# kfjahnke/envutil

Hardware: AMD Instinct MI355X
Metric: Mpix/s reprojected (16K lat/lon->cubemap, b-spline-3) (higher is better)
Workload: dtype f32

## Files before the change

### envutil_amd/csrc/eu_render4.hip

```cpp
#include <cstdlib>
#include <cstdio>
#include <cstring>
#include <vector>
#include <algorithm>
#include "eu_packed_dev.h"

#define EU4_TW 16
#define EU4_TH 8
#define EU4_WAVES 4
#ifndef EU4_WAVES0
#define EU4_WAVES0 1
#define EU4_TEXELS 384
#define EU4_OCC0 4
#endif
#define EU4_SHARDS 1024
#define EU4_WL_SHARD(s) (16 * (s))
#define EU4_WL_DONE1 (16 * EU4_SHARDS)
#define EU4_WL_DYN(x) (16 * (EU4_SHARDS + 1 + (x)))
#define EU4_WL_ENTRIES (16 * (EU4_SHARDS + 16))
#define EU4_UNIT_ROWS 4
#define EU4_COL_FLOATS 8
#define EU4_MAX_PLANS 16

__device__ __forceinline__ void eu4_box_reduce(int &mn0, int &mn1, int &mx0, int &mx1)
{
#define EU4_RED(ctrl)                                        \
  "v_min_i32_dpp %0, %0, %0 " ctrl "\n\t"                    \
  "v_min_i32_dpp %1, %1, %1 " ctrl "\n\t"                    \
  "v_max_i32_dpp %2, %2, %2 " ctrl "\n\t"                    \
  "v_max_i32_dpp %3, %3, %3 " ctrl "\n\t"
  asm("s_nop 1\n\t"
      EU4_RED("row_shr:1 row_mask:0xf bank_mask:0xf")
      EU4_RED("row_shr:2 row_mask:0xf bank_mask:0xf")
      EU4_RED("row_shr:4 row_mask:0xf bank_mask:0xf")
      EU4_RED("row_shr:8 row_mask:0xf bank_mask:0xf")
      EU4_RED("row_bcast:15 row_mask:0xa bank_mask:0xf")
      EU4_RED("row_bcast:31 row_mask:0xc bank_mask:0xf")
      "s_nop 0"
      : "+v"(mn0), "+v"(mn1), "+v"(mx0), "+v"(mx1));
#undef EU4_RED
  mn0 = __builtin_amdgcn_readlane(mn0, 63); mn1 = __builtin_amdgcn_readlane(mn1, 63);
  mx0 = __builtin_amdgcn_readlane(mx0, 63); mx1 = __builtin_amdgcn_readlane(mx1, 63);
}

typedef __attribute__((address_space(3))) void *eu4_lds_void;
typedef const __attribute__((address_space(1))) void *eu4_gbl_void;

typedef float eu4_f4 __attribute__((ext_vector_type(4)));

__device__ __forceinline__ void eu4_dma_row(unsigned dst, unsigned voff, const char *sb)
{
  unsigned keep;
  asm volatile("s_mov_b32 %0, m0\n\t"
               "s_mov_b32 m0, %1\n\t"
               "s_nop 0\n\t"
               "global_load_lds_dwordx4 %2, %3\n\t"
               "s_mov_b32 m0, %0"
               : "=&s"(keep) : "s"(dst), "v"(voff), "s"(sb) : "memory");
}

struct eu4_plan {
  const float *atab_g;
  const int *tileplan;
  const float *coltab;
  int tiles16;
  const int *l2_rows;
  int l2_off[9];
  int l2_half;
  unsigned long long l2_magic;
  const int *l1_rows;
  int l1_off[9];
  unsigned long long l1_magic;
#ifdef EU5_STAMPS
  unsigned long long *stamps;
#endif
};

#ifdef EU5_STAMPS
#define EU5_STAMP(k) do { asm volatile("" ::: "memory"); st_[k] = __builtin_amdgcn_s_memtime(); asm volatile("" ::: "memory"); } while (0)
#else
#define EU5_STAMP(k) do { } while (0)
#endif

template <int NCH, int DEG, int PRJ>
__device__ __forceinline__ void eu4_tile(const eu_render_params &p, const eu4_plan &w, const float *atab,
                                         float *wtile, int tile_y, int x0, int lane)
{
  constexpr int TEX = 4;
  constexpr int order = DEG + 1;
  const eu_src_dev &s = p.src;
  const int lx = lane & 7, ly = lane >> 3;
  const int y = p.row_begin + tile_y * EU4_TH + ly;
  const bool yin = y < p.row_end;
  const int yc = yin ? y : p.row_end - 1;
  const float *rt = p.row + (long long)eu_frame_row(yc, p.band_shift, p.band_count, p.band_index) * EU_ROW_FLOATS;
  const int xa = x0 + 2 * lx, xb = xa + 1;
  const bool va = yin && xa < p.width, vb = yin && xb < p.width;
  const int xac = xa < p.width ? xa : p.width - 1, xbc = xb < p.width ? xb : p.width - 1;

  eu_f2 tx, ty, gy;
  eu_i2 hit, ok = { -1, -1 };
  int ixa, ixb;
  float wxa[order], wxb[order];
  eu_ray2 r;
  {
    const float A0 = rt[0], A1 = rt[1], A2 = rt[2], B0 = rt[3], B1 = rt[4], B2 = rt[5];
    const eu_f2 c0 = { p.col[xac], p.col[xbc] };
    if (p.form == EU_FORM_BCA) {
      const float C0 = rt[6], C1 = rt[7], C2 = rt[8];
      const float *colB = p.col + p.width;
      const eu_f2 c1 = { colB[xac], colB[xbc] };
      r.x = B0 * c0 + C0 * c1 + A0;
      r.y = B1 * c0 + C1 * c1 + A1;
      r.z = B2 * c0 + C2 * c1 + A2;
    } else {
      r.x = B0 * c0 + A0;
      r.y = B1 * c0 + A1;
      r.z = B2 * c0 + A2;
    }
    if (p.norm_mode == EU_NORM_DIV) {
      eu_f2 sqn = r.x * r.x; sqn = sqn + r.y * r.y; sqn = sqn + r.z * r.z;
      const eu_f2 n = { sqrtf(sqn.x), sqrtf(sqn.y) };
      r.x = r.x / n; r.y = r.y / n; r.z = r.z / n;
    }
  }
  asm volatile("s_waitcnt vmcnt(0)" ::: "memory");
  eu_f2 sx, sy;
  hit = eu_coord2_ok<PRJ>(s, r, sx, sy, atab, ok);
  const eu_f2 gx = eu_gate2_ok(sx, s.gate0, s.lower0, s.upper0, ok);
  gy = eu_gate2_ok(sy, s.gate1, s.lower1, s.upper1, ok);
  eu_f2 fx;
  if constexpr (DEG & 1) fx = (eu_f2){ floorf(gx.x), floorf(gx.y) };
  else fx = (eu_f2){ roundf(gx.x), roundf(gx.y) };
  tx = gx - fx;
  ixa = (int)fx.x; ixb = (int)fx.y;
  hit = hit & (eu_i2){ va ? -1 : 0, vb ? -1 : 0 };
  eu_f2 fy;
  if constexpr (DEG & 1) fy = (eu_f2){ floorf(gy.x), floorf(gy.y) };
  else fy = (eu_f2){ roundf(gy.x), roundf(gy.y) };
  ty = gy - fy;
  const int iya = (int)fy.x, iyb = (int)fy.y;

  int mnx = INT_MAX, mny = INT_MAX, mxx = INT_MIN, mxy = INT_MIN;
  if (hit.x) { mnx = ixa; mxx = ixa; mny = iya; mxy = iya; }
  if (hit.y) { mnx = min(mnx, ixb); mxx = max(mxx, ixb); mny = min(mny, iyb); mxy = max(mxy, iyb); }
  eu4_box_reduce(mnx, mny, mxx, mxy);
  const bool any = mnx != INT_MAX;
  const long long bw = (long long)mxx - mnx + order, bh = (long long)mxy - mny + order;
  const bool fits = bw <= 64 && bh <= EU4_TEXELS && bw * bh <= EU4_TEXELS;
  const bool clean = __ballot((hit.x && !ok.x) || (hit.y && !ok.y)) == 0ull;
  float *const orow = p.out + (long long)(yc - p.row_begin) * p.out_stride;
  if (any && !(fits && clean)) {
    if (lane == 0) {
      const int id = tile_y * w.tiles16 + x0 / EU4_TW;
      const int sh = (int)(((unsigned)id * 0x9E3779B1u) >> 22) & (EU4_SHARDS - 1);
      const int slot = atomicAdd(p.wl + EU4_WL_SHARD(sh), 1);
      p.wl[EU4_WL_ENTRIES + (size_t)slot * EU4_SHARDS + sh] = id;
    }
    return;
  }
  float qa[NCH], qb[NCH];
  if (any) {
    const int ibw = (int)bw, ibh = (int)bh;
    const unsigned lds_tile = (unsigned)(unsigned long long)(eu4_lds_void)wtile;
    if (lane < ibw) {
      const int bx0 = mnx - DEG / 2, by0 = mny - DEG / 2;
      const unsigned voff = (unsigned)(lane * NCH) * 4u;
      const char *sb = (const char *)(s.base + ((long long)by0 * s.es1 + (long long)bx0 * NCH));
      const long long step = s.es1 * 4;
      unsigned dst = lds_tile;
      const unsigned dstep = (unsigned)ibw * (TEX * 4u);
#pragma unroll 1
      for (int it = 0; it < ibh; it++) { eu4_dma_row(dst, voff, sb); sb += step; dst += dstep; }
    }
    eu_f2 wx[order], wy[order];
    float wya[order], wyb[order];
    if constexpr (DEG >= 2) {
      eu_weights2<DEG>(s.wm, ty, wy);
      eu_weights2<DEG>(s.wm, tx, wx);
    }
#pragma unroll
    for (int i = 0; i < order; i++) {
      if constexpr (DEG >= 2) {
        wya[i] = wy[i].x; wyb[i] = wy[i].y;
        wxa[i] = wx[i].x; wxb[i] = wx[i].y;
      } else {
        wya[i] = wyb[i] = 0.0f;
        wxa[i] = wxb[i] = 0.0f;
      }
    }
    const int oa = hit.x ? ((iya - mny) * ibw + (ixa - mnx)) * TEX : 0;
    const int ob = hit.y ? ((iyb - mny) * ibw + (ixb - mnx)) * TEX : 0;
    asm volatile("s_waitcnt vmcnt(0)" ::: "memory");
    eu_lptr lt = (eu_lptr)wtile;
    eu_accumulate1<NCH, DEG, TEX, int, eu_lptr>(lt + oa, ibw * TEX, wxa, wya, tx.x, ty.x, qa);
    eu_accumulate1<NCH, DEG, TEX, int, eu_lptr>(lt + ob, ibw * TEX, wxb, wyb, tx.y, ty.y, qb);
  } else {
#pragma unroll
    for (int c = 0; c < NCH; c++) { qa[c] = 0.0f; qb[c] = 0.0f; }
  }
  constexpr int ncol = (NCH == 2 || NCH == 4) ? NCH - 1 : NCH;
  const bool bright = s.brighten != 1.0f;
#pragma unroll
  for (int c = 0; c < NCH; c++) {
    float a = qa[c], bb = qb[c];
    if (bright && c < ncol) { a = a * s.brighten; bb = bb * s.brighten; }
    qa[c] = hit.x ? a : 0.0f;
    qb[c] = hit.y ? bb : 0.0f;
  }
  if (va) eu_put<NCH>(orow, xa, qa);
  if (vb) eu_put<NCH>(orow, xb, qb);
}

template <int NCH, int DEG, int PRJ>
__global__ __launch_bounds__(64 * EU4_WAVES0, EU4_OCC0) void eu_render4s_kernel(const eu_render_params p, const eu4_plan w)
{
  __shared__ __attribute__((aligned(16))) float tile_all[EU4_WAVES0 * EU4_TEXELS * 4];
  __shared__ __attribute__((aligned(16))) float atab[768];
  const int lane = threadIdx.x & 63;
  const int wave = __builtin_amdgcn_readfirstlane(threadIdx.x >> 6);
  float *const tile = tile_all + wave * (EU4_TEXELS * 4);
  if (PRJ != EU_CUBEMAP && wave == 0) {
    static_assert(EU_ATAN_TAB_FLOATS * 4 <= 3 * 1024, "three pieces");
#pragma unroll
    for (int i = 0; i < 3; i++)
      __builtin_amdgcn_global_load_lds((eu4_gbl_void)(w.atab_g + i * 256 + lane * 4),
                                       (eu4_lds_void)(atab + i * 256), 16, 0, 0);
  }
  const int tile_x = (int)(blockIdx.x >> 3) * EU4_WAVES0 + wave;
  const int tile_y = ((int)blockIdx.z * 8 + (int)(blockIdx.x & 7)) * EU4_UNIT_ROWS + (int)blockIdx.y;
  if (tile_y >= p.tiles_y) return;
  if constexpr (EU4_WAVES0 > 1) {
    asm volatile("s_waitcnt vmcnt(0)" ::: "memory");
    __syncthreads();
  }
  if (tile_x >= w.tiles16) return;
  eu4_tile<NCH, DEG, PRJ>(p, w, atab, tile, tile_y, tile_x * EU4_TW, lane);
}

template <int NCH, int DEG, int PRJ>
__device__ __forceinline__ void eu4_direct_tile(const eu_render_params &p, const float *atab, int tile_y, int x0, int lane)
{
  const eu_src_dev &s = p.src;
  const int lx = lane & 7, ly = lane >> 3;
  const int y = p.row_begin + tile_y * EU4_TH + ly;
  const bool yin = y < p.row_end;
  const int yc = yin ? y : p.row_end - 1;
  const float *rt = p.row + (long long)eu_frame_row(yc, p.band_shift, p.band_count, p.band_index) * EU_ROW_FLOATS;
  const int xa = x0 + 2 * lx, xb = xa + 1;
  const bool va = yin && xa < p.width, vb = yin && xb < p.width;
  const int xac = xa < p.width ? xa : p.width - 1, xbc = xb < p.width ? xb : p.width - 1;
  eu_ray2 ry;
  {
    const float A0 = rt[0], A1 = rt[1], A2 = rt[2], B0 = rt[3], B1 = rt[4], B2 = rt[5];
    const eu_f2 c0 = { p.col[xac], p.col[xbc] };
    if (p.form == EU_FORM_BCA) {
      const float C0 = rt[6], C1 = rt[7], C2 = rt[8];
      const float *colB = p.col + p.width;
      const eu_f2 c1 = { colB[xac], colB[xbc] };
      ry.x = B0 * c0 + C0 * c1 + A0;
      ry.y = B1 * c0 + C1 * c1 + A1;
      ry.z = B2 * c0 + C2 * c1 + A2;
    } else {
      ry.x = B0 * c0 + A0;
      ry.y = B1 * c0 + A1;
      ry.z = B2 * c0 + A2;
    }
    if (p.norm_mode == EU_NORM_DIV) {
      eu_f2 sqn = ry.x * ry.x; sqn = sqn + ry.y * ry.y; sqn = sqn + ry.z * ry.z;
      const eu_f2 n = { sqrtf(sqn.x), sqrtf(sqn.y) };
      ry.x = ry.x / n; ry.y = ry.y / n; ry.z = ry.z / n;
    }
  }
  eu_f2 sx, sy;
  eu_i2 hit = eu_coord2<PRJ>(s, ry, sx, sy, atab);
  hit = hit & (eu_i2){ va ? -1 : 0, vb ? -1 : 0 };
  float pxa[NCH], pxb[NCH];
  eu_eval2<NCH, DEG>(s, sx, sy, hit, pxa, pxb);
  float *const orow = p.out + (long long)(yc - p.row_begin) * p.out_stride;
  if (va) eu_put<NCH>(orow, xa, pxa);
  if (vb) eu_put<NCH>(orow, xb, pxb);
}

#include "eu_render5.h"

template <int DEG>
__global__ __launch_bounds__(256) void eu_colplan_kernel(const eu_render_params p, float *ct,
                                                         float A0, float A2, float B0, float B2)
{
  __shared__ __attribute__((aligned(16))) float atab[EU_ATAN_TAB_FLOATS];
  if (threadIdx.x < EU_ATAN_TAB_ENTRIES) eu_atan_tab_entry(threadIdx.x, atab + 8 * threadIdx.x);
  __syncthreads();
  constexpr int order = DEG + 1;
  const eu_src_dev &s = p.src;
  const int xa = 2 * (blockIdx.x * 256 + threadIdx.x), xb = xa + 1;
  if (xa >= p.width) return;
  const int xbc = xb < p.width ? xb : p.width - 1;
  const eu_f2 c0 = { p.col[xa], p.col[xbc] };
  const eu_f2 rx = B0 * c0 + A0, rz = B2 * c0 + A2;
  eu_i2 ok = { -1, -1 };
  const eu_f2 q2 = rx * rx + rz * rz;
  const eu_f2 qs = eu_sqrt2_ok(q2, ok);
  const eu_f2 lon = eu_atan2f_2_tab_ok(rx, rz, atab, 0, ok);
  eu_f2 i0 = { (float)((double)lon.x - s.tex_x0), (float)((double)lon.y - s.tex_x0) };
  if (s.cdiv_ok) i0 = eu_div2_const(i0, s.ext_w, s.rcp_ext_w);
  else i0 = i0 / s.ext_w;
  i0 = i0 * s.total_w; i0 = i0 - .5f;
  const eu_f2 sx = i0 - s.win_x_off;
  const eu_f2 gx = eu_gate2_ok(sx, s.gate0, s.lower0, s.upper0, ok);
  eu_f2 fx;
  if constexpr (DEG & 1) fx = (eu_f2){ floorf(gx.x), floorf(gx.y) };
  else fx = (eu_f2){ roundf(gx.x), roundf(gx.y) };
  const eu_f2 tx = gx - fx;
  eu_f2 wx[4];
#pragma unroll
  for (int i = 0; i < 4; i++) wx[i] = (eu_f2){ 0.0f, 0.0f };
  if constexpr (DEG >= 2) eu_weights2<DEG>(s.wm, tx, wx);
  float e[2][EU4_COL_FLOATS];
  e[0][0] = __int_as_float(ok.x ? (int)fx.x : INT_MIN);
  e[1][0] = __int_as_float(ok.y ? (int)fx.y : INT_MIN);
  e[0][1] = tx.x; e[1][1] = tx.y;
#pragma unroll
  for (int i = 0; i < 4; i++) { e[0][2 + i] = i < order ? wx[i].x : 0.0f; e[1][2 + i] = i < order ? wx[i].y : 0.0f; }
  e[0][6] = qs.x; e[1][6] = qs.y;
  e[0][7] = lon.x; e[1][7] = lon.y;
  float *o = ct + (size_t)xa * EU4_COL_FLOATS;
#pragma unroll
  for (int i = 0; i < EU4_COL_FLOATS; i++) o[i] = e[0][i];
  if (xb < p.width) {
#pragma unroll
    for (int i = 0; i < EU4_COL_FLOATS; i++) o[EU4_COL_FLOATS + i] = e[1][i];
  }
}

template <int NCH, int DEG, int PRJ>
__global__ __launch_bounds__(256, 4) void eu_render4d_kernel(const eu_render_params p, const eu4_plan w)
{
  __shared__ __attribute__((aligned(16))) float atab[EU_ATAN_TAB_FLOATS];
  if constexpr (PRJ != EU_CUBEMAP) {
    if (threadIdx.x < EU_ATAN_TAB_ENTRIES) eu_atan_tab_entry(threadIdx.x, atab + 8 * threadIdx.x);
  }
  const int lane = threadIdx.x & 63;
  const int wave = __builtin_amdgcn_readfirstlane(threadIdx.x >> 6);
  const int gid = blockIdx.x * EU4_WAVES + wave;
  const int sh = gid & (EU4_SHARDS - 1);
  const int nwork = __builtin_amdgcn_readfirstlane(
    __hip_atomic_load(p.wl + EU4_WL_SHARD(sh), __ATOMIC_RELAXED, __HIP_MEMORY_SCOPE_AGENT));
  __syncthreads();
#pragma unroll 1
  for (int k = gid / EU4_SHARDS; k < nwork; k += (int)(gridDim.x * EU4_WAVES / EU4_SHARDS)) {
    const int id = __builtin_amdgcn_readfirstlane(p.wl[EU4_WL_ENTRIES + (size_t)k * EU4_SHARDS + sh]);
    const int tile_y = id / w.tiles16;
    const int x0 = (id - tile_y * w.tiles16) * EU4_TW;
    eu4_direct_tile<NCH, DEG, PRJ>(p, atab, tile_y, x0, lane);
  }
  __shared__ int last;
  __syncthreads();
  if (threadIdx.x == 0) last = atomicAdd(p.wl + EU4_WL_DONE1, 1) == (int)gridDim.x - 1;
  __syncthreads();
  if (last) {
    for (int i = threadIdx.x; i <= EU4_SHARDS + 8; i += 256)
      __hip_atomic_store(p.wl + 16 * i, 0, __ATOMIC_RELAXED, __HIP_MEMORY_SCOPE_AGENT);
  }
}

#ifndef EU4_DIRECT_WGS
#define EU4_DIRECT_WGS 2048
#endif

template <int NCH, int DEG, int PRJ>
static int launch4_ndp(const eu_render_params &p, const eu4_plan &w, hipStream_t st)
{
  if constexpr (PRJ == EU_SPHERICAL) {
    static const int cus = [] {
      int dev = 0, n = 0;
      if (hipGetDevice(&dev) != hipSuccess) return 0;
      if (hipDeviceGetAttribute(&n, hipDeviceAttributeMultiprocessorCount, dev) != hipSuccess) return 0;
      return n;
    }();
    auto mag_ok = [](double v) { const double a = v < 0 ? -v : v; return a == 0.0 || (a >= 0x1p-20 && a <= 0x1p20); };
    const bool fast = p.form == EU_FORM_BA && p.norm_mode == EU_NORM_NONE && p.band_count <= 1 && p.src.brighten == 1.0f &&
                      p.src.always_hit && mag_ok(p.src.tex_x0) && mag_ok(p.src.tex_y0) && p.src.ext_w >= 0x1p-20f &&
                      p.src.ext_w <= 0x1p20f && p.src.ext_h >= 0x1p-20f && p.src.ext_h <= 0x1p20f && p.tab_finite;
    int per_cu = 0;
    if (fast) {
      static const int occ = [] { int n = 0; return hipOccupancyMaxActiveBlocksPerMultiprocessor(&n, eu_render5_kernel<NCH, DEG, PRJ, true>, 64 * EU5_WAVES, 0) == hipSuccess ? n : 0; }();
      per_cu = occ;
    } else {
      static const int occ = [] { int n = 0; return hipOccupancyMaxActiveBlocksPerMultiprocessor(&n, eu_render5_kernel<NCH, DEG, PRJ, false>, 64 * EU5_WAVES, 0) == hipSuccess ? n : 0; }();
      per_cu = occ;
    }
    const int wgs = (cus / 8) * 8 * per_cu;
    if (wgs <= 0) return -1;
    if (fast) hipLaunchKernelGGL((eu_render5_kernel<NCH, DEG, PRJ, true>), dim3((unsigned)wgs), dim3(64 * EU5_WAVES), 0, st, p, w);
    else hipLaunchKernelGGL((eu_render5_kernel<NCH, DEG, PRJ, false>), dim3((unsigned)wgs), dim3(64 * EU5_WAVES), 0, st, p, w);
  } else {
    const int units = (p.tiles_y + EU4_UNIT_ROWS - 1) / EU4_UNIT_ROWS;
    dim3 grid((unsigned)(8 * ((w.tiles16 + EU4_WAVES0 - 1) / EU4_WAVES0)), (unsigned)EU4_UNIT_ROWS, (unsigned)((units + 7) / 8));
    hipLaunchKernelGGL((eu_render4s_kernel<NCH, DEG, PRJ>), grid, dim3(64 * EU4_WAVES0), 0, st, p, w);
  }
  if (hipGetLastError() != hipSuccess) return -1;
  hipLaunchKernelGGL((eu_render4d_kernel<NCH, DEG, PRJ>), dim3(EU4_DIRECT_WGS), dim3(256), 0, st, p, w);
  if (hipGetLastError() != hipSuccess) {
    (void)hipMemsetAsync(p.wl, 0, EU4_WL_ENTRIES * sizeof(int), st);
    return -1;
  }
  return 0;
}

template <int NCH, int DEG>
static int launch4_nd(const eu_render_params &p, const eu4_plan &w, hipStream_t st)
{
  switch (p.src.prj) {
    case EU_SPHERICAL: return launch4_ndp<NCH, DEG, EU_SPHERICAL>(p, w, st);
    case EU_CUBEMAP: return launch4_ndp<NCH, DEG, EU_CUBEMAP>(p, w, st);
    case EU_BIATAN6: return launch4_ndp<NCH, DEG, EU_BIATAN6>(p, w, st);
  }
  return 1;
}

template <int NCH>
static int launch4_n(const eu_render_params &p, const eu4_plan &w, hipStream_t st)
{
  switch (p.src.degree) {
    case 1: return launch4_nd<NCH, 1>(p, w, st);
    case 2: return launch4_nd<NCH, 2>(p, w, st);
    case 3: return launch4_nd<NCH, 3>(p, w, st);
  }
  return 1;
}

extern "C" size_t eu_render4_worklist_ints(size_t ntiles)
{
  return EU4_WL_ENTRIES + ((ntiles + EU4_SHARDS - 1) / EU4_SHARDS) * EU4_SHARDS;
}
extern "C" size_t eu_render4_worklist_header_ints(void) { return EU4_WL_ENTRIES; }

extern "C" int eu_current_slot(void);
namespace {
struct plan_cache {
  std::vector<unsigned char> key;
  int *tileplan = nullptr; size_t tileplan_cap = 0;
  float *coltab = nullptr; size_t coltab_cap = 0;
  float *atab = nullptr;
  int planned_rows = 0;
  int *l2_rows = nullptr; size_t l2_cap = 0;
  int l2_off[9] = {};
  int *l1_rows = nullptr; size_t l1_cap = 0;
  int l1_off[9] = {};
  hipStream_t last_stream = nullptr;
} g4s[EU_MAX_SLOTS];
#define g4 (g4s[eu_current_slot()])

bool ensure_atab()
{
  if (g4.atab) return true;
  std::vector<float> tab(768, 0.0f);
  for (int i = 0; i < EU_ATAN_TAB_ENTRIES; i++) eu_atan_tab_entry(i, tab.data() + 8 * i);
  if (hipMalloc((void **)&g4.atab, tab.size() * sizeof(float)) != hipSuccess) return false;
  return hipMemcpy(g4.atab, tab.data(), tab.size() * sizeof(float), hipMemcpyHostToDevice) == hipSuccess;
}

template <int DEG>
void launch_colplan(const eu_render_params &p, float *ct, const float *k, hipStream_t st)
{
  hipLaunchKernelGGL((eu_colplan_kernel<DEG>), dim3((unsigned)((p.width + 511) / 512)), dim3(256), 0, st, p, ct,
                     k[0], k[1], k[2], k[3]);
}
}

extern "C" int eu_launch_render4(const eu_render_params *pp, const float *h_row, size_t h_row_floats,
                                 unsigned long long plan_gen, int only_if_worth, void *stream)
{
  eu_render_params p = *pp;
  if (p.twine || p.stage != 0 || p.form >= EU_FORM_FISH || p.src.has_lcp || p.nch_out != p.nch) return 1;
  if (p.norm_mode != EU_NORM_NONE && p.norm_mode != EU_NORM_DIV) return 1;
  if (p.src.prj != EU_SPHERICAL && p.src.prj != EU_CUBEMAP && p.src.prj != EU_BIATAN6) return 1;
  if (p.src.degree < 1 || p.src.degree > 3 || p.src.es0 != p.nch) return 1;
  if (p.nch != 3 && p.nch != 4) return 1;
  if (!p.wl) return 1;
  if (p.src.es1 * 4 >= (1ll << 31)) return 1;
  p.tiles_y = (p.row_end - p.row_begin + EU4_TH - 1) / EU4_TH;
  eu4_plan w;
  w.tiles16 = (p.width + EU4_TW - 1) / EU4_TW;
  if (w.tiles16 <= 0 || p.tiles_y <= 0) return 0;
  if (p.tiles_y > 65535 * 8 * EU4_UNIT_ROWS) return 1;
  hipStream_t st = (hipStream_t)stream;
  if (!ensure_atab()) return -1;
  w.atab_g = g4.atab;

  std::vector<unsigned char> key(sizeof(unsigned long long) + sizeof(eu_src_dev) + 8 * sizeof(int));
  {
    unsigned char *q = key.data();
    memcpy(q, &plan_gen, sizeof plan_gen); q += sizeof plan_gen;
    eu_src_dev sd = p.src; sd.base = nullptr;
    memcpy(q, &sd, sizeof sd); q += sizeof sd;
    const int v[8] = { p.width, p.row_begin, p.row_end, p.band_shift, p.band_count, p.band_index, p.form, p.norm_mode };
    memcpy(q, v, sizeof v);
  }
  if (p.src.prj == EU_SPHERICAL && key != g4.key) {
    std::vector<int> tp((size_t)p.tiles_y, -1);
    std::vector<float> plans;
    const bool can = p.src.prj == EU_SPHERICAL && p.form == EU_FORM_BA && p.norm_mode == EU_NORM_NONE && h_row;
    static const bool off = [] { const char *e = getenv("EU_HIP_COLPLAN"); return e && e[0] == '0'; }();
    if (can && !off) {
      for (int ty = 0; ty < p.tiles_y; ty++) {
        float k[4] = { 0, 0, 0, 0 };
        bool same = true;
        for (int ly = 0; ly < EU4_TH && same; ly++) {
          const int y = std::min(p.row_begin + ty * EU4_TH + ly, p.row_end - 1);
          const size_t fr = (size_t)eu_frame_row(y, p.band_shift, p.band_count, p.band_index) * EU_ROW_FLOATS;
          if (fr + 6 > h_row_floats) { same = false; break; }
          const float c[4] = { h_row[fr + 0], h_row[fr + 2], h_row[fr + 3], h_row[fr + 5] };
          if (ly == 0) memcpy(k, c, sizeof k);
          else same = memcmp(k, c, sizeof k) == 0;
        }
        if (!same) continue;
        int id = -1;
        for (size_t j = 0; j < plans.size() / 4 && id < 0; j++)
          if (memcmp(&plans[4 * j], k, sizeof k) == 0) id = (int)j;
        if (id < 0 && plans.size() / 4 < EU4_MAX_PLANS) {
          id = (int)(plans.size() / 4);
          plans.insert(plans.end(), k, k + 4);
        }
        tp[(size_t)ty] = id;
      }
    }
    if (g4.tileplan_cap < tp.size()) {
      if (g4.tileplan) (void)hipFree(g4.tileplan);
      g4.tileplan = nullptr; g4.tileplan_cap = 0;
      if (hipMalloc((void **)&g4.tileplan, tp.size() * sizeof(int)) != hipSuccess) return -1;
      g4.tileplan_cap = tp.size();
    }
    const size_t need = std::max<size_t>(1, plans.size() / 4) * (size_t)p.width * EU4_COL_FLOATS;
    if (g4.coltab_cap < need) {
      if (g4.coltab) (void)hipFree(g4.coltab);
      g4.coltab = nullptr; g4.coltab_cap = 0;
      if (hipMalloc((void **)&g4.coltab, need * sizeof(float)) != hipSuccess) return -1;
      g4.coltab_cap = need;
    }
    if (hipStreamSynchronize(st) != hipSuccess) return -1;
    if (g4.last_stream && g4.last_stream != st && hipStreamSynchronize(g4.last_stream) != hipSuccess) return -1;
    if (hipMemcpy(g4.tileplan, tp.data(), tp.size() * sizeof(int), hipMemcpyHostToDevice) != hipSuccess) return -1;
    g4.planned_rows = 0;
    for (int v : tp) g4.planned_rows += v >= 0;
    {
      std::vector<int> rows[8];
      for (int r = 0; r < p.tiles_y; r++) {
        const int m = r >> 1;
        const bool paired = 2 * m + 1 < p.tiles_y && tp[(size_t)2 * m] >= 0 && tp[(size_t)2 * m] == tp[(size_t)2 * m + 1];
        if (!paired) rows[(r / EU5_UNIT_ROWS) & 7].push_back(r);
      }
      std::vector<int> all;
      for (int x = 0; x < 8; x++) { g4.l2_off[x] = (int)all.size(); all.insert(all.end(), rows[x].begin(), rows[x].end()); }
      g4.l2_off[8] = (int)all.size();
      if (g4.l2_cap < all.size() + 1) {
        if (g4.l2_rows) (void)hipFree(g4.l2_rows);
        g4.l2_rows = nullptr; g4.l2_cap = 0;
        if (hipMalloc((void **)&g4.l2_rows, (all.size() + 1) * sizeof(int)) != hipSuccess) return -1;
        g4.l2_cap = all.size() + 1;
      }
      if (!all.empty() && hipMemcpy(g4.l2_rows, all.data(), all.size() * sizeof(int), hipMemcpyHostToDevice) != hipSuccess) return -1;
      std::vector<int> prs[8];
      for (int m = 0; 2 * m + 1 < p.tiles_y; m++)
        if (tp[(size_t)2 * m] >= 0 && tp[(size_t)2 * m] == tp[(size_t)2 * m + 1]) {
          auto &v = prs[(m / (EU5_UNIT_ROWS / 2)) & 7];
          v.push_back(m); v.push_back(tp[(size_t)2 * m]);
        }
      std::vector<int> all1;
      for (int x = 0; x < 8; x++) { g4.l1_off[x] = (int)all1.size() / 2; all1.insert(all1.end(), prs[x].begin(), prs[x].end()); }
      g4.l1_off[8] = (int)all1.size() / 2;
      if (g4.l1_cap < all1.size() + 2) {
        if (g4.l1_rows) (void)hipFree(g4.l1_rows);
        g4.l1_rows = nullptr; g4.l1_cap = 0;
        if (hipMalloc((void **)&g4.l1_rows, (all1.size() + 2) * sizeof(int)) != hipSuccess) return -1;
        g4.l1_cap = all1.size() + 2;
      }
      if (!all1.empty() && hipMemcpy(g4.l1_rows, all1.data(), all1.size() * sizeof(int), hipMemcpyHostToDevice) != hipSuccess) return -1;
    }
    for (size_t j = 0; j < plans.size() / 4; j++) {
      float *ct = g4.coltab + j * (size_t)p.width * EU4_COL_FLOATS;
      switch (p.src.degree) {
        case 1: launch_colplan<1>(p, ct, &plans[4 * j], st); break;
        case 2: launch_colplan<2>(p, ct, &plans[4 * j], st); break;
        default: launch_colplan<3>(p, ct, &plans[4 * j], st); break;
      }
      if (hipGetLastError() != hipSuccess) return -1;
    }
    g4.key.swap(key);
  }
  if (only_if_worth && p.src.prj == EU_SPHERICAL) {
    if (p.src.degree < 2 || g4.planned_rows * 2 < p.tiles_y) return 1;
  }
  w.tileplan = g4.tileplan;
  w.coltab = g4.coltab;
  w.l2_rows = g4.l2_rows;
  for (int x = 0; x < 9; x++) w.l2_off[x] = g4.l2_off[x];
  w.l2_half = (w.tiles16 + 1) / 2;
  w.l2_magic = (1ull << 40) / (unsigned long long)w.l2_half + 1;
  w.l1_rows = g4.l1_rows;
  for (int x = 0; x < 9; x++) w.l1_off[x] = g4.l1_off[x];
  w.l1_magic = (1ull << 40) / (unsigned long long)w.tiles16 + 1;
  g4.last_stream = st;
#ifdef EU5_STAMPS
  static unsigned long long *d_st = nullptr; static size_t st_cap = 0; static int dumps = 0;
  const size_t ntile_st = (size_t)w.tiles16 * p.tiles_y * 8;
  const size_t nst = ntile_st + 8192 * 4;
  if (st_cap < nst) { if (d_st) (void)hipFree(d_st); if (hipMalloc((void **)&d_st, nst * 8) != hipSuccess) return -1; st_cap = nst; }
  (void)hipMemsetAsync(d_st, 0, nst * 8, st);
  w.stamps = d_st;
  int rc_ = p.nch == 3 ? launch4_n<3>(p, w, st) : p.nch == 4 ? launch4_n<4>(p, w, st) : 1;
  if (rc_ == 0 && dumps < 2 && nst >= 8 * 4096) {
    dumps++;
    std::vector<unsigned long long> h(nst);
    (void)hipStreamSynchronize(st);
    (void)hipMemcpy(h.data(), d_st, nst * 8, hipMemcpyDeviceToHost);
    double acc[32][8] = {}; size_t cnt[32] = {};
    for (size_t t = 0; t < ntile_st / 8; t++) {
      const unsigned long long *q = &h[t * 8];
      if (!q[0] || !q[7]) continue;
      const int cls = (int)(q[1] & 31);
      cnt[cls]++;
      acc[cls][0] += (double)(q[2] - q[0]); acc[cls][1] += (double)(q[3] - q[2]);
      if (q[4]) { acc[cls][2] += (double)(q[4] - q[3]); acc[cls][3] += (double)(q[5] - q[4]); acc[cls][4] += (double)(q[6] - q[5]); }
      acc[cls][5] += (double)(q[7] - q[6]); acc[cls][6] += (double)(q[7] - q[0]);
    }
    {
      double mn = 1e30, mx = 0, sum = 0, l1 = 0, first = 1e30, last = 0; size_t nw = 0;
      for (size_t k = 0; k < 8192; k++) {
        const unsigned long long *q = &h[ntile_st + k * 4];
        if (!q[3]) continue;
        const double d = (double)(q[2] - q[0]);
        mn = std::min(mn, d); mx = std::max(mx, d); sum += d; l1 += (double)(q[1] - q[0]); nw++;
        first = std::min(first, (double)q[0]); last = std::max(last, (double)q[2]);
      }
      if (nw) fprintf(stderr, "eu5 waves: %zu, cycles per wave min %.0f avg %.0f max %.0f, first loop avg %.0f, first start .. last end %.0f\n",
                      nw, mn, sum / nw, mx, l1 / nw, last - first);
    }
    for (int c = 0; c < 32; c++) if (cnt[c])
      fprintf(stderr, "eu5 stamps: hoist %d npass %2d tiles %8zu | coords %7.0f box %6.0f dma-issue+weights %6.0f dma-wait %6.0f taps(all passes) %6.0f store %5.0f | tile %7.0f (100 MHz ticks? s_memtime)\n",
              c >> 4, (c & 15) - 1, cnt[c], acc[c][0] / cnt[c], acc[c][1] / cnt[c], acc[c][2] / cnt[c], acc[c][3] / cnt[c], acc[c][4] / cnt[c], acc[c][5] / cnt[c], acc[c][6] / cnt[c]);
  }
  return rc_;
#else
  switch (p.nch) {
    case 3: return launch4_n<3>(p, w, st);
    case 4: return launch4_n<4>(p, w, st);
  }
  return 1;
#endif
}
```

### envutil_amd/csrc/eu_render5.h

```cpp
#define EU5_WAVES 4
#ifndef EU5_TEXELS
#define EU5_TEXELS 576
#endif
#ifndef EU5_OCC
#define EU5_OCC 4
#endif
#ifndef EU5_UNIT_ROWS
#define EU5_UNIT_ROWS 4
#endif

__device__ __forceinline__ int eu4_shard_of(int id)
{
  return (int)(((unsigned)id * 0x9E3779B1u) >> 22) & (EU4_SHARDS - 1);
}

typedef const __attribute__((address_space(3))) eu4_f4 *eu5_l4ptr;

template <int NCH, int DEG>
__device__ __forceinline__ void eu5_taps(eu_lptr lt, int a, int b, int pitch, const eu_f2 *wx, const eu_f2 *wy,
                                         eu_f2 tx, eu_f2 ty, eu_f2 &rga, eu_f2 &bxa, eu_f2 &rgb, eu_f2 &bxb)
{
  constexpr int order = DEG + 1;
  if constexpr (DEG == 1) {
    const eu_f2 wl0 = 1.0f - tx, wr0 = tx, wl1 = 1.0f - ty, wr1 = ty;
    const eu4_f4 a00 = *(eu5_l4ptr)(lt + a), a01 = *(eu5_l4ptr)(lt + a + 4);
    const eu4_f4 a10 = *(eu5_l4ptr)(lt + a + pitch), a11 = *(eu5_l4ptr)(lt + a + pitch + 4);
    const eu4_f4 b00 = *(eu5_l4ptr)(lt + b), b01 = *(eu5_l4ptr)(lt + b + 4);
    const eu4_f4 b10 = *(eu5_l4ptr)(lt + b + pitch), b11 = *(eu5_l4ptr)(lt + b + pitch + 4);
    {
      const eu_f2 l0 = { wl0.x, wl0.x }, r0 = { wr0.x, wr0.x }, l1 = { wl1.x, wl1.x }, r1 = { wr1.x, wr1.x };
      eu_f2 s = a00.xy * l0; s = s + a01.xy * r0; s = s * l1;
      eu_f2 u = a10.xy * l0; u = u + a11.xy * r0; rga = s + u * r1;
      s = a00.zw * l0; s = s + a01.zw * r0; s = s * l1;
      u = a10.zw * l0; u = u + a11.zw * r0; bxa = s + u * r1;
    }
    {
      const eu_f2 l0 = { wl0.y, wl0.y }, r0 = { wr0.y, wr0.y }, l1 = { wl1.y, wl1.y }, r1 = { wr1.y, wr1.y };
      eu_f2 s = b00.xy * l0; s = s + b01.xy * r0; s = s * l1;
      eu_f2 u = b10.xy * l0; u = u + b11.xy * r0; rgb = s + u * r1;
      s = b00.zw * l0; s = s + b01.zw * r0; s = s * l1;
      u = b10.zw * l0; u = u + b11.zw * r0; bxb = s + u * r1;
    }
  } else {
#pragma unroll
    for (int j = 0; j < order; j++) {
      eu4_f4 ta[order], tb[order];
#pragma unroll
      for (int i = 0; i < order; i++) {
        ta[i] = *(eu5_l4ptr)(lt + a + j * pitch + 4 * i);
        tb[i] = *(eu5_l4ptr)(lt + b + j * pitch + 4 * i);
      }
      const eu_f2 w0a = { wx[0].x, wx[0].x }, w0b = { wx[0].y, wx[0].y };
      eu_f2 ra = ta[0].xy * w0a, qa = ta[0].zw * w0a, rb = tb[0].xy * w0b, qb = tb[0].zw * w0b;
#pragma unroll
      for (int i = 1; i < order; i++) {
        const eu_f2 wa = { wx[i].x, wx[i].x }, wb = { wx[i].y, wx[i].y };
        ra = EU_MAD2(wa, ta[i].xy, ra); qa = EU_MAD2(wa, ta[i].zw, qa);
        rb = EU_MAD2(wb, tb[i].xy, rb); qb = EU_MAD2(wb, tb[i].zw, qb);
      }
      const eu_f2 ya = { wy[j].x, wy[j].x }, yb = { wy[j].y, wy[j].y };
      if (j == 0) { rga = ra * ya; bxa = qa * ya; rgb = rb * yb; bxb = qb * yb; }
      else { rga = EU_MAD2(ra, ya, rga); bxa = EU_MAD2(qa, ya, bxa); rgb = EU_MAD2(rb, yb, rgb); bxb = EU_MAD2(qb, yb, bxb); }
    }
  }
}

__device__ __forceinline__ void eu5_box_reduce(int &q0, int &q1, int &q2, int &q3, int &h0, int &h1, int &h2, int &h3)
{
#define EU5_RED(ctrl)                                        \
  "v_min_i32_dpp %0, %0, %0 " ctrl "\n\t"                    \
  "v_min_i32_dpp %1, %1, %1 " ctrl "\n\t"                    \
  "v_max_i32_dpp %2, %2, %2 " ctrl "\n\t"                    \
  "v_max_i32_dpp %3, %3, %3 " ctrl "\n\t"
  asm("s_nop 1\n\t"
      EU5_RED("row_shr:1 row_mask:0xf bank_mask:0xf")
      EU5_RED("row_shr:2 row_mask:0xf bank_mask:0xf")
      EU5_RED("row_shr:4 row_mask:0xf bank_mask:0xf")
      EU5_RED("row_shr:8 row_mask:0xf bank_mask:0xf")
      "v_mov_b32 %4, %0\n\tv_mov_b32 %5, %1\n\tv_mov_b32 %6, %2\n\tv_mov_b32 %7, %3\n\t"
      "v_min_i32_dpp %4, %0, %4 row_bcast:15 row_mask:0xa bank_mask:0xf\n\t"
      "v_min_i32_dpp %5, %1, %5 row_bcast:15 row_mask:0xa bank_mask:0xf\n\t"
      "v_max_i32_dpp %6, %2, %6 row_bcast:15 row_mask:0xa bank_mask:0xf\n\t"
      "v_max_i32_dpp %7, %3, %7 row_bcast:15 row_mask:0xa bank_mask:0xf\n\t"
      "s_nop 0"
      : "+v"(q0), "+v"(q1), "+v"(q2), "+v"(q3), "=&v"(h0), "=&v"(h1), "=&v"(h2), "=&v"(h3));
#undef EU5_RED
}

struct eu5_box { int mnx, mny, mxx, mxy; };

struct eu5_divtab_t { unsigned v[65]; };
static constexpr eu5_divtab_t eu5_make_divtab()
{
  eu5_divtab_t t = {};
  t.v[0] = 0;
  for (unsigned w = 1; w <= 64; w++) t.v[w] = ((65536u + w - 1) / w) | ((64u / w) << 24);
  return t;
}
__constant__ const eu5_divtab_t eu5_divtab = eu5_make_divtab();

__device__ __forceinline__ eu5_box eu5_box_at(int a, int b, int c, int d, int lane)
{
  eu5_box r;
  r.mnx = __builtin_amdgcn_readlane(a, lane); r.mny = __builtin_amdgcn_readlane(b, lane);
  r.mxx = __builtin_amdgcn_readlane(c, lane); r.mxy = __builtin_amdgcn_readlane(d, lane);
  return r;
}
__device__ __forceinline__ eu5_box eu5_box_join(const eu5_box &a, const eu5_box &b)
{
  eu5_box r = { min(a.mnx, b.mnx), min(a.mny, b.mny), max(a.mxx, b.mxx), max(a.mxy, b.mxy) };
  return r;
}
template <int ORDER>
__device__ __forceinline__ int eu5_box_fits(const eu5_box &b)
{
  if (b.mnx == INT_MAX) return -1;
  const unsigned bw = (unsigned)b.mxx - (unsigned)b.mnx + ORDER, bh = (unsigned)b.mxy - (unsigned)b.mny + ORDER;
  return bw <= 64u && bh <= (unsigned)EU5_TEXELS && bw * bh <= (unsigned)EU5_TEXELS;
}

__device__ __forceinline__ eu_f2 eu5_gate2(eu_f2 c, int kind, float lower, float upper)
{
  if (kind == 0) {
    eu_f2 r = c;
    r = eu_sel2(c < lower, (eu_f2){ lower, lower }, r);
    r = eu_sel2(c > upper, (eu_f2){ upper, upper }, r);
    return r;
  }
  eu_f2 cc = c - lower;
  if (kind == 1) cc = eu_abs2(cc);
  return cc + lower;
}

__device__ __forceinline__ int eu5_out_of_range3(float a, float b, float c)
{
  const float hi = __builtin_fmaxf(__builtin_fmaxf(__builtin_fabsf(a), __builtin_fabsf(b)), __builtin_fabsf(c));
  const float lo = __builtin_fminf(__builtin_fminf(__builtin_fabsf(a), __builtin_fabsf(b)), __builtin_fabsf(c));
  return (hi <= 0x1p40f && lo >= 0x1p-40f) ? 0 : -1;
}

struct eu5_tab8 { eu_f2 c0; float A0, A1, A2, B0, B1, B2; };

template <bool FAST>
__device__ __forceinline__ void eu5_load8(const eu_render_params &p, int tile_y, int x0, int lane, eu5_tab8 &T)
{
  const int pr = lane & 3, rw = (lane >> 2) & 7, hf = lane >> 5;
  const int y = p.row_begin + tile_y * EU4_TH + rw;
  const int yc = y < p.row_end ? y : p.row_end - 1;
  const float *rt = p.row + (long long)(FAST ? yc : eu_frame_row(yc, p.band_shift, p.band_count, p.band_index)) * EU_ROW_FLOATS;
  const int xa = x0 + 8 * hf + 2 * pr, xb = xa + 1;
  const int xac = xa < p.width ? xa : p.width - 1, xbc = xb < p.width ? xb : p.width - 1;
  T.A0 = rt[0]; T.A1 = rt[1]; T.A2 = rt[2]; T.B0 = rt[3]; T.B1 = rt[4]; T.B2 = rt[5];
  T.c0 = (eu_f2){ p.col[xac], p.col[xbc] };
}

template <int NCH, int DEG, int PRJ, bool HOIST, bool FAST, bool PRE = false>
__device__ __forceinline__ void eu5_tile(const eu_render_params &p, const eu4_plan &w, const float *atab,
                                         float *wtile, const float *ct, int tile_y, int x0, int lane,
                                         const eu5_tab8 *T = nullptr, bool have_n = false, int ty_n = 0, int x0_n = 0,
                                         eu5_tab8 *Tn = nullptr)
{
  static_assert(!PRE || (!HOIST && FAST), "the prefetching form exists for plain FAST tiles");
  constexpr int TEX = 4;
  constexpr int order = DEG + 1;
  const eu_src_dev &s = p.src;
#ifdef EU5_STAMPS
  unsigned long long st_[8] = { 0, 0, 0, 0, 0, 0, 0, 0 };
#endif
  EU5_STAMP(0);
  const int pr = lane & 3, rw = (lane >> 2) & 7, hf = lane >> 5;
  const int y = p.row_begin + tile_y * EU4_TH + rw;
  const bool yin = y < p.row_end;
  const int yc = yin ? y : p.row_end - 1;
  const float *rt = p.row + (long long)(FAST ? yc : eu_frame_row(yc, p.band_shift, p.band_count, p.band_index)) * EU_ROW_FLOATS;
  const int xa = x0 + 8 * hf + 2 * pr, xb = xa + 1;
  const bool va = yin && xa < p.width, vb = yin && xb < p.width;
  const int xac = xa < p.width ? xa : p.width - 1, xbc = xb < p.width ? xb : p.width - 1;

  eu_f2 tx, ty, gy;
  eu_i2 hit, ok = { -1, -1 };
  int ixa, ixb;
  eu_f2 wx[order], wy[order];
  constexpr bool LEAN = FAST && PRJ == EU_SPHERICAL;
  if constexpr (LEAN) {
    hit = (eu_i2){ -1, -1 };
    eu_i2 big0 = { 0, 0 }, big1 = { 0, 0 };
    eu_f2 lat;
    if constexpr (HOIST) {
      const float4 *ea = (const float4 *)(ct + (size_t)xac * EU4_COL_FLOATS);
      const float4 *eb = (const float4 *)(ct + (size_t)xbc * EU4_COL_FLOATS);
      const float4 a0 = ea[0], a1 = ea[1], b0 = eb[0], b1 = eb[1];
      const float A1 = rt[1], B1 = rt[4];
      const eu_f2 c0 = { p.col[xac], p.col[xbc] };
      const eu_f2 ryy = B1 * c0 + A1;
      ixa = __float_as_int(a0.x); ixb = __float_as_int(b0.x);
      tx = (eu_f2){ a0.y, b0.y };
      if constexpr (DEG >= 2) {
        wx[0] = (eu_f2){ a0.z, b0.z }; wx[1] = (eu_f2){ a0.w, b0.w }; wx[2] = (eu_f2){ a1.x, b1.x };
        if constexpr (DEG == 3) wx[3] = (eu_f2){ a1.y, b1.y };
      }
      const eu_f2 qs = { a1.z, b1.z };
      ok = (eu_i2){ (ixa != INT_MIN ? -1 : 0) & ~eu5_out_of_range3(ryy.x, qs.x, qs.x),
                    (ixb != INT_MIN ? -1 : 0) & ~eu5_out_of_range3(ryy.y, qs.y, qs.y) };
      lat = eu_atan2f_2_lean(ryy, qs, atab, 1, big0);
    } else {
      float A0, A1, A2, B0, B1, B2;
      eu_f2 c0;
      if constexpr (PRE) { A0 = T->A0; A1 = T->A1; A2 = T->A2; B0 = T->B0; B1 = T->B1; B2 = T->B2; c0 = T->c0; }
      else {
        A0 = rt[0]; A1 = rt[1]; A2 = rt[2]; B0 = rt[3]; B1 = rt[4]; B2 = rt[5];
        c0 = (eu_f2){ p.col[xac], p.col[xbc] };
      }
      const eu_f2 rx = B0 * c0 + A0, ry = B1 * c0 + A1, rz = B2 * c0 + A2;
      ok = (eu_i2){ ~eu5_out_of_range3(rx.x, ry.x, rz.x), ~eu5_out_of_range3(rx.y, ry.y, rz.y) };
      const eu_f2 q2 = rx * rx + rz * rz;
      const eu_f2 qs = eu_sqrt2_safe(q2);
      lat = eu_atan2f_2_lean(ry, qs, atab, 1, big0);
      const eu_f2 lon = eu_atan2f_2_lean(rx, rz, atab, 0, big1);
      eu_f2 i0 = { (float)((double)lon.x - s.tex_x0), (float)((double)lon.y - s.tex_x0) };
      if (s.cdiv_ok) i0 = eu_div2_const(i0, s.ext_w, s.rcp_ext_w);
      else i0 = eu_div2_rr(i0, s.ext_w, eu_rcp_refined(s.ext_w));
      i0 = i0 * s.total_w; i0 = i0 - .5f;
      const eu_f2 sx = i0 - s.win_x_off;
      const eu_f2 gx = eu5_gate2(sx, s.gate0, s.lower0, s.upper0);
      eu_f2 fx;
      if constexpr (DEG & 1) fx = (eu_f2){ floorf(gx.x), floorf(gx.y) };
      else fx = (eu_f2){ roundf(gx.x), roundf(gx.y) };
      tx = gx - fx;
      ixa = (int)fx.x; ixb = (int)fx.y;
    }
    ok = ok & ~(big0 | big1);
    eu_f2 i1 = { (float)((double)lat.x - s.tex_y0), (float)((double)lat.y - s.tex_y0) };
    if (s.cdiv_ok) i1 = eu_div2_const(i1, s.ext_h, s.rcp_ext_h);
    else i1 = eu_div2_rr(i1, s.ext_h, eu_rcp_refined(s.ext_h));
    i1 = i1 * s.total_h; i1 = i1 - .5f;
    const eu_f2 sy = i1 - s.win_y_off;
    gy = eu5_gate2(sy, s.gate1, s.lower1, s.upper1);
  } else if constexpr (HOIST) {
    const float4 *ea = (const float4 *)(ct + (size_t)xac * EU4_COL_FLOATS);
    const float4 *eb = (const float4 *)(ct + (size_t)xbc * EU4_COL_FLOATS);
    const float4 a0 = ea[0], a1 = ea[1], b0 = eb[0], b1 = eb[1];
    const float A1 = rt[1], B1 = rt[4];
    const eu_f2 c0 = { p.col[xac], p.col[xbc] };
    const eu_f2 ryy = B1 * c0 + A1;
    ixa = __float_as_int(a0.x); ixb = __float_as_int(b0.x);
    ok = ok & (eu_i2){ ixa != INT_MIN ? -1 : 0, ixb != INT_MIN ? -1 : 0 };
    tx = (eu_f2){ a0.y, b0.y };
    if constexpr (DEG >= 2) {
      wx[0] = (eu_f2){ a0.z, b0.z }; wx[1] = (eu_f2){ a0.w, b0.w }; wx[2] = (eu_f2){ a1.x, b1.x };
      if constexpr (DEG == 3) wx[3] = (eu_f2){ a1.y, b1.y };
    }
    const eu_f2 qs = { a1.z, b1.z };
    const eu_f2 lat = eu_atan2f_2_tab_ok(ryy, qs, atab, 1, ok);
    hit = (eu_i2){ -1, -1 };
    if (!FAST && !s.always_hit) {
      const eu_f2 lon = { a1.w, b1.w };
      hit = (lon >= s.wex0) & (lon <= s.wex1) & (lat >= s.wex2) & (lat <= s.wex3);
    }
    eu_f2 i1 = { (float)((double)lat.x - s.tex_y0), (float)((double)lat.y - s.tex_y0) };
    if (FAST || s.cdiv_ok) i1 = eu_div2_const(i1, s.ext_h, s.rcp_ext_h);
    else i1 = i1 / s.ext_h;
    i1 = i1 * s.total_h; i1 = i1 - .5f;
    const eu_f2 sy = i1 - s.win_y_off;
    gy = eu_gate2_ok(sy, s.gate1, s.lower1, s.upper1, ok);
  } else {
    eu_ray2 r;
    {
      float A0, A1, A2, B0, B1, B2;
      eu_f2 c0;
      if constexpr (PRE) { A0 = T->A0; A1 = T->A1; A2 = T->A2; B0 = T->B0; B1 = T->B1; B2 = T->B2; c0 = T->c0; }
      else {
        A0 = rt[0]; A1 = rt[1]; A2 = rt[2]; B0 = rt[3]; B1 = rt[4]; B2 = rt[5];
        c0 = (eu_f2){ p.col[xac], p.col[xbc] };
      }
      if (!FAST && p.form == EU_FORM_BCA) {
        const float C0 = rt[6], C1 = rt[7], C2 = rt[8];
        const float *colB = p.col + p.width;
        const eu_f2 c1 = { colB[xac], colB[xbc] };
        r.x = B0 * c0 + C0 * c1 + A0;
        r.y = B1 * c0 + C1 * c1 + A1;
        r.z = B2 * c0 + C2 * c1 + A2;
      } else {
        r.x = B0 * c0 + A0;
        r.y = B1 * c0 + A1;
        r.z = B2 * c0 + A2;
      }
      if (!FAST && p.norm_mode == EU_NORM_DIV) {
        eu_f2 sqn = r.x * r.x; sqn = sqn + r.y * r.y; sqn = sqn + r.z * r.z;
        const eu_f2 n = { sqrtf(sqn.x), sqrtf(sqn.y) };
        r.x = r.x / n; r.y = r.y / n; r.z = r.z / n;
      }
    }
    eu_f2 sx, sy;
    hit = eu_coord2_ok<PRJ, FAST>(s, r, sx, sy, atab, ok);
    const eu_f2 gx = eu_gate2_ok(sx, s.gate0, s.lower0, s.upper0, ok);
    gy = eu_gate2_ok(sy, s.gate1, s.lower1, s.upper1, ok);
    eu_f2 fx;
    if constexpr (DEG & 1) fx = (eu_f2){ floorf(gx.x), floorf(gx.y) };
    else fx = (eu_f2){ roundf(gx.x), roundf(gx.y) };
    tx = gx - fx;
    ixa = (int)fx.x; ixb = (int)fx.y;
  }
  hit = hit & (eu_i2){ va ? -1 : 0, vb ? -1 : 0 };
  eu_f2 fy;
  if constexpr (DEG & 1) fy = (eu_f2){ floorf(gy.x), floorf(gy.y) };
  else fy = (eu_f2){ roundf(gy.x), roundf(gy.y) };
  ty = gy - fy;
  const int iya = (int)fy.x, iyb = (int)fy.y;
#ifdef EU5_STAMPS
  asm volatile("" : : "v"(iya), "v"(iyb), "v"(ixa), "v"(ixb));
#endif
  EU5_STAMP(2);

  int q0 = INT_MAX, q1 = INT_MAX, q2 = INT_MIN, q3 = INT_MIN, h0, h1, h2, h3;
  if (hit.x) { q0 = ixa; q2 = ixa; q1 = iya; q3 = iya; }
  if (hit.y) { q0 = min(q0, ixb); q2 = max(q2, ixb); q1 = min(q1, iyb); q3 = max(q3, iyb); }
  eu5_box_reduce(q0, q1, q2, q3, h0, h1, h2, h3);
  const eu5_box full = eu5_box_join(eu5_box_at(h0, h1, h2, h3, 31), eu5_box_at(h0, h1, h2, h3, 63));
  bool clean = __ballot((hit.x && !ok.x) || (hit.y && !ok.y)) == 0ull;
  if constexpr (LEAN) {
    const int cw = (int)(s.upper0 + 0.5f), ch = (int)(s.upper1 + 0.5f);
    if (full.mnx != INT_MAX) {
      if (s.gate0 == 2 && full.mnx < 0) clean = false;
      if (s.gate0 != 0 && full.mxx >= cw - 1) clean = false;
      if (s.gate1 == 2 && full.mny < 0) clean = false;
      if (s.gate1 != 0 && full.mxy >= ch - 1) clean = false;
    }
  }
  int npass = 1;
  const int f = eu5_box_fits<order>(full);
  if (f < 0) npass = 0;
  else if (f == 0) {
    npass = 2;
    if (eu5_box_fits<order>(eu5_box_at(h0, h1, h2, h3, 31)) == 0 || eu5_box_fits<order>(eu5_box_at(h0, h1, h2, h3, 63)) == 0) {
      npass = 4;
      if (eu5_box_fits<order>(eu5_box_at(q0, q1, q2, q3, 15)) == 0 || eu5_box_fits<order>(eu5_box_at(q0, q1, q2, q3, 31)) == 0 ||
          eu5_box_fits<order>(eu5_box_at(q0, q1, q2, q3, 47)) == 0 || eu5_box_fits<order>(eu5_box_at(q0, q1, q2, q3, 63)) == 0)
        npass = -1;
    }
  }
  EU5_STAMP(3);
  float *const orow = p.out + (long long)(yc - p.row_begin) * p.out_stride;
  if (npass < 0 || (npass > 0 && !clean)) {
    if (lane == 0) {
      const int id = tile_y * w.tiles16 + x0 / EU4_TW;
      const int sh = eu4_shard_of(id);
      const int slot = atomicAdd(p.wl + EU4_WL_SHARD(sh), 1);
      p.wl[EU4_WL_ENTRIES + (size_t)slot * EU4_SHARDS + sh] = id;
    }
    if constexpr (PRE) { if (have_n) eu5_load8<FAST>(p, ty_n, x0_n, lane, *Tn); }
    return;
  }
  eu_f2 rga = { 0.0f, 0.0f }, bxa = { 0.0f, 0.0f }, rgb = { 0.0f, 0.0f }, bxb = { 0.0f, 0.0f };
  if (npass > 0) {
    const unsigned lds_tile = (unsigned)(unsigned long long)(eu4_lds_void)wtile;
    const int grp = npass == 1 ? 0 : npass == 2 ? hf : (lane >> 4);
#pragma unroll 1
    for (int pi = 0; pi < npass; pi++) {
      eu5_box bx = full;
      if (npass > 1) {
        const int ln = npass == 2 ? 31 + 32 * pi : 15 + 16 * pi;
        const eu5_box bh = eu5_box_at(h0, h1, h2, h3, ln), bq = eu5_box_at(q0, q1, q2, q3, ln);
        bx = npass == 2 ? bh : bq;
      }
      if (bx.mnx == INT_MAX) continue;
      const int ibw = bx.mxx - bx.mnx + order, ibh = bx.mxy - bx.mny + order;
      {
        const unsigned tv = eu5_divtab.v[ibw];
        const int k = (int)(tv >> 24);
        const unsigned r = ((unsigned)lane * (tv & 0x1ffffu)) >> 16, c = (unsigned)lane - r * (unsigned)ibw;
        const int bx0 = bx.mnx - DEG / 2, by0 = bx.mny - DEG / 2;
        const unsigned pitchb = (unsigned)(s.es1 * 4);
        const unsigned voff = r * pitchb + c * (NCH * 4u);
        const char *sb = (const char *)(s.base + ((long long)by0 * s.es1 + (long long)bx0 * NCH));
        const unsigned long long step = (unsigned long long)k * pitchb;
        unsigned dst = lds_tile;
        const unsigned dstep = (unsigned)(k * ibw) * (TEX * 4u);
        int left = ibh;
        if ((int)r < k) {
#pragma unroll 1
          for (; left >= k; left -= k) { eu4_dma_row(dst, voff, sb); sb += step; dst += dstep; }
        }
        left = ibh % k;
        if ((int)r < left) {
          const int full = ibh / k;
          eu4_dma_row(lds_tile + (unsigned)full * dstep, voff,
                      (const char *)(s.base + ((long long)by0 * s.es1 + (long long)bx0 * NCH)) + (unsigned long long)full * step);
        }
      }
      if (pi == 0) {
        if constexpr (DEG >= 2) {
          eu_weights2<DEG>(s.wm, ty, wy);
          if constexpr (!HOIST) eu_weights2<DEG>(s.wm, tx, wx);
        }
      }
      const bool mine = grp == pi;
      const int oa = (mine && hit.x) ? ((iya - bx.mny) * ibw + (ixa - bx.mnx)) * TEX : 0;
      const int ob = (mine && hit.y) ? ((iyb - bx.mny) * ibw + (ixb - bx.mnx)) * TEX : 0;
      if (pi == 0) EU5_STAMP(4);
      asm volatile("s_waitcnt vmcnt(0)" ::: "memory");
      if (pi == 0) EU5_STAMP(5);
      if (mine) eu5_taps<NCH, DEG>((eu_lptr)wtile, oa, ob, ibw * TEX, wx, wy, tx, ty, rga, bxa, rgb, bxb);
    }
  }
#ifdef EU5_STAMPS
  asm volatile("" : : "v"(rga), "v"(bxa), "v"(rgb), "v"(bxb));
#endif
  EU5_STAMP(6);
  float qa[4] = { rga.x, rga.y, bxa.x, bxa.y }, qb[4] = { rgb.x, rgb.y, bxb.x, bxb.y };
  constexpr int ncol = (NCH == 2 || NCH == 4) ? NCH - 1 : NCH;
  const bool bright = !FAST && s.brighten != 1.0f;
#pragma unroll
  for (int c = 0; c < NCH; c++) {
    float a = qa[c], bb = qb[c];
    if (bright && c < ncol) { a = a * s.brighten; bb = bb * s.brighten; }
    qa[c] = hit.x ? a : 0.0f;
    qb[c] = hit.y ? bb : 0.0f;
  }
  if constexpr (PRE) {
    if (have_n) eu5_load8<FAST>(p, ty_n, x0_n, lane, *Tn);
    __builtin_amdgcn_sched_barrier(0);
  }
  if (va) eu_put<NCH>(orow, xa, qa);
  if (vb) eu_put<NCH>(orow, xb, qb);
  EU5_STAMP(7);
#ifdef EU5_STAMPS
  if (lane == 0 && w.stamps) {
    unsigned long long *o = w.stamps + ((size_t)tile_y * w.tiles16 + x0 / EU4_TW) * 8;
    st_[1] = (unsigned long long)(npass + 1) | (HOIST ? 16ull : 0ull);
#pragma unroll
    for (int k = 0; k < 8; k++) o[k] = st_[k];
  }
#endif
}



template <int NCH, int DEG>
__device__ __forceinline__ void eu5_stage(const eu_src_dev &s, const eu5_box &bx, unsigned lds_tile, int lane)
{
  constexpr int order = DEG + 1;
  const int ibw = bx.mxx - bx.mnx + order, ibh = bx.mxy - bx.mny + order;
  const unsigned tv = eu5_divtab.v[ibw];
  const int k = (int)(tv >> 24);
  const unsigned r = ((unsigned)lane * (tv & 0x1ffffu)) >> 16, c = (unsigned)lane - r * (unsigned)ibw;
  const int bx0 = bx.mnx - DEG / 2, by0 = bx.mny - DEG / 2;
  const unsigned pitchb = (unsigned)(s.es1 * 4);
  const unsigned voff = r * pitchb + c * (NCH * 4u);
  const char *const sb0 = (const char *)(s.base + ((long long)by0 * s.es1 + (long long)bx0 * NCH));
  const unsigned long long step = (unsigned long long)k * pitchb;
  const unsigned dstep = (unsigned)(k * ibw) * 16u;
  if ((int)r < k) {
    const char *sb = sb0;
    unsigned dst = lds_tile;
#pragma unroll 1
    for (int left = ibh; left >= k; left -= k) { eu4_dma_row(dst, voff, sb); sb += step; dst += dstep; }
  }
  if ((int)r < ibh % k) {
    const int full = ibh / k;
    eu4_dma_row(lds_tile + (unsigned)full * dstep, voff, sb0 + (unsigned long long)full * step);
  }
}

struct eu5_tab16 {
  eu4_f4 a0, a1, b0, b1;
  eu_f2 c0;
  float A1A, B1A, A1B, B1B;
};

__device__ __forceinline__ void eu5_load16(const eu_render_params &p, const float *ct, int tile_y, int x0, int lane, eu5_tab16 &T)
{
  const int pr = lane & 3, rw = (lane >> 2) & 7, hf = lane >> 5;
  const int yA = p.row_begin + tile_y * EU4_TH + rw, yB = yA + EU4_TH;
  const int ycA = yA < p.row_end ? yA : p.row_end - 1, ycB = yB < p.row_end ? yB : p.row_end - 1;
  const float *rtA = p.row + (long long)ycA * EU_ROW_FLOATS, *rtB = p.row + (long long)ycB * EU_ROW_FLOATS;
  const int xa = x0 + 8 * hf + 2 * pr, xb = xa + 1;
  const int xac = xa < p.width ? xa : p.width - 1, xbc = xb < p.width ? xb : p.width - 1;
  const eu4_f4 *ea = (const eu4_f4 *)(ct + (size_t)xac * EU4_COL_FLOATS);
  const eu4_f4 *eb = (const eu4_f4 *)(ct + (size_t)xbc * EU4_COL_FLOATS);
  T.a0 = ea[0]; T.a1 = ea[1]; T.b0 = eb[0]; T.b1 = eb[1];
  T.A1A = rtA[1]; T.B1A = rtA[4]; T.A1B = rtB[1]; T.B1B = rtB[4];
  T.c0 = (eu_f2){ p.col[xac], p.col[xbc] };
}

template <int NCH, int DEG>
__device__ __forceinline__ bool eu5_tile16h(const eu_render_params &p, const eu4_plan &w, const float *atab,
                                            float *wtile, const eu5_tab16 &T, int tile_y, int x0, int lane,
                                            bool have_n, const float *ct_n, int ty_n, int x0_n, eu5_tab16 &Tn)
{
  constexpr int order = DEG + 1;
  const eu_src_dev &s = p.src;
#ifdef EU5_STAMPS
  unsigned long long st_[8] = { 0, 0, 0, 0, 0, 0, 0, 0 };
#endif
  EU5_STAMP(0);
  const int pr = lane & 3, rw = (lane >> 2) & 7, hf = lane >> 5;
  const int yA = p.row_begin + tile_y * EU4_TH + rw, yB = yA + EU4_TH;
  const bool yinA = yA < p.row_end, yinB = yB < p.row_end;
  const int ycA = yinA ? yA : p.row_end - 1, ycB = yinB ? yB : p.row_end - 1;
  const int xa = x0 + 8 * hf + 2 * pr, xb = xa + 1;
  const bool vxa = xa < p.width, vxb = xb < p.width;
  const eu4_f4 a0 = T.a0, a1 = T.a1, b0 = T.b0, b1 = T.b1;
  const eu_f2 c0 = T.c0;
  const eu_f2 ryA = T.B1A * c0 + T.A1A, ryB = T.B1B * c0 + T.A1B;
  const int ixa = __float_as_int(a0.x), ixb = __float_as_int(b0.x);
  eu_f2 wx[order];
  const eu_f2 tx = { a0.y, b0.y };
  if constexpr (DEG >= 2) {
    wx[0] = (eu_f2){ a0.z, b0.z }; wx[1] = (eu_f2){ a0.w, b0.w }; wx[2] = (eu_f2){ a1.x, b1.x };
    if constexpr (DEG == 3) wx[3] = (eu_f2){ a1.y, b1.y };
  }
  const eu_f2 qs = { a1.z, b1.z };
  eu_i2 bigA = { 0, 0 }, bigB = { 0, 0 };
  int bad = ((ixa != INT_MIN && ixb != INT_MIN) ? 0 : -1) |
            eu5_out_of_range3(ryA.x, qs.x, ryB.x) | eu5_out_of_range3(ryA.y, qs.y, ryB.y);
  const eu_f2 latA = eu_atan2f_2_lean(ryA, qs, atab, 1, bigA);
  const eu_f2 latB = eu_atan2f_2_lean(ryB, qs, atab, 1, bigB);
  bad |= bigA.x | bigA.y | bigB.x | bigB.y;
  const float rr = s.cdiv_ok ? 0.0f : eu_rcp_refined(s.ext_h);
  eu_f2 iA = { (float)((double)latA.x - s.tex_y0), (float)((double)latA.y - s.tex_y0) };
  eu_f2 iB = { (float)((double)latB.x - s.tex_y0), (float)((double)latB.y - s.tex_y0) };
  if (s.cdiv_ok) { iA = eu_div2_const(iA, s.ext_h, s.rcp_ext_h); iB = eu_div2_const(iB, s.ext_h, s.rcp_ext_h); }
  else { iA = eu_div2_rr(iA, s.ext_h, rr); iB = eu_div2_rr(iB, s.ext_h, rr); }
  iA = iA * s.total_h; iA = iA - .5f; iB = iB * s.total_h; iB = iB - .5f;
  const eu_f2 gyA = eu5_gate2(iA - s.win_y_off, s.gate1, s.lower1, s.upper1);
  const eu_f2 gyB = eu5_gate2(iB - s.win_y_off, s.gate1, s.lower1, s.upper1);
  eu_f2 fyA, fyB;
  if constexpr (DEG & 1) { fyA = (eu_f2){ floorf(gyA.x), floorf(gyA.y) }; fyB = (eu_f2){ floorf(gyB.x), floorf(gyB.y) }; }
  else { fyA = (eu_f2){ roundf(gyA.x), roundf(gyA.y) }; fyB = (eu_f2){ roundf(gyB.x), roundf(gyB.y) }; }
  const eu_f2 tyA = gyA - fyA, tyB = gyB - fyB;
  const int iyAa = (int)fyA.x, iyAb = (int)fyA.y, iyBa = (int)fyB.x, iyBb = (int)fyB.y;
  const bool hAa = yinA && vxa, hAb = yinA && vxb, hBa = yinB && vxa, hBb = yinB && vxb;

#ifdef EU5_STAMPS
  asm volatile("" : : "v"(iyAa), "v"(iyAb), "v"(iyBa), "v"(iyBb));
#endif
  EU5_STAMP(2);
  int q0 = INT_MAX, q1 = INT_MAX, q2 = INT_MIN, q3 = INT_MIN, h0, h1, h2, h3;
  if (hAa) { q0 = ixa; q2 = ixa; q1 = iyAa; q3 = iyAa; }
  if (hAb) { q0 = min(q0, ixb); q2 = max(q2, ixb); q1 = min(q1, iyAb); q3 = max(q3, iyAb); }
  if (hBa) { q0 = min(q0, ixa); q2 = max(q2, ixa); q1 = min(q1, iyBa); q3 = max(q3, iyBa); }
  if (hBb) { q0 = min(q0, ixb); q2 = max(q2, ixb); q1 = min(q1, iyBb); q3 = max(q3, iyBb); }
  eu5_box_reduce(q0, q1, q2, q3, h0, h1, h2, h3);
  eu5_box bx = eu5_box_join(eu5_box_at(h0, h1, h2, h3, 31), eu5_box_at(h0, h1, h2, h3, 63));
  bool fast = __ballot(bad != 0 && (hAa || hAb || hBa || hBb)) == 0ull;
  if (bx.mnx != INT_MAX) {
    const int cw = (int)(s.upper0 + 0.5f), ch = (int)(s.upper1 + 0.5f);
    if (s.gate0 == 2 && bx.mnx < 0) fast = false;
    if (s.gate0 != 0 && bx.mxx >= cw - 1) fast = false;
    if (s.gate1 == 2 && bx.mny < 0) fast = false;
    if (s.gate1 != 0 && bx.mxy >= ch - 1) fast = false;
    if (eu5_box_fits<order>(bx) != 1) fast = false;
  }
  if (bx.mnx == INT_MAX || !fast) {
    if (have_n) eu5_load16(p, ct_n, ty_n, x0_n, lane, Tn);
    return bx.mnx == INT_MAX;
  }
  bx.mnx = __builtin_amdgcn_readfirstlane(bx.mnx); bx.mny = __builtin_amdgcn_readfirstlane(bx.mny);
  bx.mxx = __builtin_amdgcn_readfirstlane(bx.mxx); bx.mxy = __builtin_amdgcn_readfirstlane(bx.mxy);
  const unsigned lds_tile = (unsigned)(unsigned long long)(eu4_lds_void)wtile;
  EU5_STAMP(3);
  eu5_stage<NCH, DEG>(s, bx, lds_tile, lane);
  eu_f2 wyA[order], wyB[order];
  if constexpr (DEG >= 2) { eu_weights2<DEG>(s.wm, tyA, wyA); eu_weights2<DEG>(s.wm, tyB, wyB); }
  const int ibw = bx.mxx - bx.mnx + order;
  const int oAa = hAa ? ((iyAa - bx.mny) * ibw + (ixa - bx.mnx)) * 4 : 0, oAb = hAb ? ((iyAb - bx.mny) * ibw + (ixb - bx.mnx)) * 4 : 0;
  const int oBa = hBa ? ((iyBa - bx.mny) * ibw + (ixa - bx.mnx)) * 4 : 0, oBb = hBb ? ((iyBb - bx.mny) * ibw + (ixb - bx.mnx)) * 4 : 0;
  EU5_STAMP(4);
  asm volatile("s_waitcnt vmcnt(0)" ::: "memory");
  EU5_STAMP(5);
  __builtin_amdgcn_sched_barrier(0);
  eu_f2 rga, bxa, rgb, bxb;
  eu5_taps<NCH, DEG>((eu_lptr)wtile, oAa, oAb, ibw * 4, wx, wyA, tx, tyA, rga, bxa, rgb, bxb);
  asm volatile("" : "+v"(rga), "+v"(bxa), "+v"(rgb), "+v"(bxb));
  {
    float qa[4] = { rga.x, rga.y, bxa.x, bxa.y }, qb[4] = { rgb.x, rgb.y, bxb.x, bxb.y };
    float *const orow = p.out + (long long)(ycA - p.row_begin) * p.out_stride;
    if (hAa) eu_put<NCH>(orow, xa, qa);
    if (hAb) eu_put<NCH>(orow, xb, qb);
  }
  EU5_STAMP(6);
  __builtin_amdgcn_sched_barrier(0);
  eu5_taps<NCH, DEG>((eu_lptr)wtile, oBa, oBb, ibw * 4, wx, wyB, tx, tyB, rga, bxa, rgb, bxb);
  asm volatile("" : "+v"(rga), "+v"(bxa), "+v"(rgb), "+v"(bxb));
  if (have_n) eu5_load16(p, ct_n, ty_n, x0_n, lane, Tn);
  __builtin_amdgcn_sched_barrier(0);
  {
    float qa[4] = { rga.x, rga.y, bxa.x, bxa.y }, qb[4] = { rgb.x, rgb.y, bxb.x, bxb.y };
    float *const orow = p.out + (long long)(ycB - p.row_begin) * p.out_stride;
    if (hBa) eu_put<NCH>(orow, xa, qa);
    if (hBb) eu_put<NCH>(orow, xb, qb);
  }
  EU5_STAMP(7);
#ifdef EU5_STAMPS
  if (lane == 0 && w.stamps) {
    unsigned long long *o = w.stamps + ((size_t)tile_y * w.tiles16 + x0 / EU4_TW) * 8;
    st_[1] = 6ull | 16ull;
#pragma unroll
    for (int k = 0; k < 8; k++) o[k] = st_[k];
  }
#endif
  return true;
}

template <int UNIT>
struct eu5_iter {
  int ul, ry, rx;
  int du, dy, dx;
  int xcd, units, tiles16;
  __device__ __forceinline__ void start(int t0, int K)
  {
    const int per_unit = UNIT * tiles16;
    ul = t0 / per_unit;
    ry = (t0 - ul * per_unit) / tiles16;
    rx = t0 - ul * per_unit - ry * tiles16;
    du = K / per_unit; dy = (K - du * per_unit) / tiles16; dx = K - du * per_unit - dy * tiles16;
  }
  __device__ __forceinline__ void step()
  {
    rx += dx; ry += dy; ul += du;
    if (rx >= tiles16) { rx -= tiles16; ry++; }
    if (ry >= UNIT) { ry -= UNIT; ul++; }
  }
  __device__ __forceinline__ bool done() const { return ul * 8 + xcd >= units; }
  __device__ __forceinline__ int row() const { return (ul * 8 + xcd) * UNIT + ry; }
  __device__ __forceinline__ int col() const
  {
    const unsigned h = ((unsigned)row() * 0x9E3779B1u) >> 16;
    int c = rx + (int)((h * (unsigned)tiles16) >> 16);
    if (c >= tiles16) c -= tiles16;
    return c;
  }
};

typedef const __attribute__((address_space(4))) int *eu5_cint;
__device__ __forceinline__ int eu5_pair_plan(const int *tileplan, int tiles_y, int m)
{
  if (2 * m + 1 >= tiles_y) return -1;
  const eu5_cint tp = (eu5_cint)tileplan;
  const int a = tp[2 * m], b = tp[2 * m + 1];
  return a == b ? a : -1;
}

template <int NCH, int DEG, int PRJ, bool FAST>
__global__ __launch_bounds__(64 * EU5_WAVES, EU5_OCC) void eu_render5_kernel(const eu_render_params p, const eu4_plan w)
{
  __shared__ __attribute__((aligned(16))) float tile_all[EU5_WAVES * EU5_TEXELS * 4];
  __shared__ __attribute__((aligned(16))) float atab[768];
  const int lane0 = threadIdx.x & 63;
  const int wave = __builtin_amdgcn_readfirstlane(threadIdx.x >> 6);
  float *const tile = tile_all + wave * (EU5_TEXELS * 4);
  if (PRJ != EU_CUBEMAP && wave == 0) {
#pragma unroll
    for (int i = 0; i < 3; i++)
      __builtin_amdgcn_global_load_lds((eu4_gbl_void)(w.atab_g + i * 256 + lane0 * 4),
                                       (eu4_lds_void)(atab + i * 256), 16, 0, 0);
    asm volatile("s_waitcnt vmcnt(0)" ::: "memory");
  }
  __syncthreads();
#ifdef EU5_STAMPS
  const unsigned long long ws0 = __builtin_amdgcn_s_memtime();
  unsigned long long ws1 = ws0;
#endif
  const int xcd = (int)(blockIdx.x & 7);
  const int K = (int)(gridDim.x >> 3) * EU5_WAVES;
  const int t0 = (int)(blockIdx.x >> 3) * EU5_WAVES + wave;
  constexpr bool PAIRS = FAST && PRJ == EU_SPHERICAL;
  if constexpr (PAIRS) {
    const int n1 = (w.l1_off[xcd + 1] - w.l1_off[xcd]) * w.tiles16;
    const eu5_cint rows1 = (eu5_cint)w.l1_rows + 2 * w.l1_off[xcd];
    int pos1 = t0;
    auto seek = [&](int &m, int &tcol, int &plan) -> bool {
      if (pos1 >= n1) return false;
      const int r = (int)(((unsigned long long)(unsigned)pos1 * w.l1_magic) >> 40);
      m = rows1[2 * r]; plan = rows1[2 * r + 1];
      const unsigned h = ((unsigned)m * 0x9E3779B1u) >> 16;
      int c = pos1 - r * w.tiles16 + (int)((h * (unsigned)w.tiles16) >> 16);
      if (c >= w.tiles16) c -= w.tiles16;
      tcol = c;
      pos1 += K;
      return true;
    };
    int m_a = 0, col_a = 0, plan_a = -1, m_b = 0, col_b = 0, plan_b = -1;
    bool have_a = seek(m_a, col_a, plan_a), have_b = false;
    eu5_tab16 Ta, Tb;
    if (have_a) eu5_load16(p, w.coltab + (size_t)plan_a * p.width * EU4_COL_FLOATS, 2 * m_a, col_a * EU4_TW, lane0, Ta);
    auto fallback = [&](int m, int tcol, int lane) {
      if (lane < 2) {
        const int id = (2 * m + lane) * w.tiles16 + tcol;
        const int sh = eu4_shard_of(id);
        const int slot = atomicAdd(p.wl + EU4_WL_SHARD(sh), 1);
        p.wl[EU4_WL_ENTRIES + (size_t)slot * EU4_SHARDS + sh] = id;
      }
    };
#pragma unroll 1
    while (have_a) {
      {
        have_b = seek(m_b, col_b, plan_b);
        int lane = lane0;
        asm volatile("" : "+v"(lane));
        const float *ct_n = w.coltab + (size_t)(have_b ? plan_b : 0) * p.width * EU4_COL_FLOATS;
        if (!eu5_tile16h<NCH, DEG>(p, w, atab, tile, Ta, 2 * m_a, col_a * EU4_TW, lane, have_b, ct_n, 2 * m_b, col_b * EU4_TW, Tb))
          fallback(m_a, col_a, lane);
      }
      if (!have_b) break;
      {
        have_a = seek(m_a, col_a, plan_a);
        int lane = lane0;
        asm volatile("" : "+v"(lane));
        const float *ct_n = w.coltab + (size_t)(have_a ? plan_a : 0) * p.width * EU4_COL_FLOATS;
        if (!eu5_tile16h<NCH, DEG>(p, w, atab, tile, Tb, 2 * m_b, col_b * EU4_TW, lane, have_a, ct_n, 2 * m_a, col_a * EU4_TW, Ta))
          fallback(m_b, col_b, lane);
      }
    }
  }
#ifdef EU5_STAMPS
  ws1 = __builtin_amdgcn_s_memtime();
#endif
  eu5_iter<EU5_UNIT_ROWS> it;
  it.xcd = xcd; it.tiles16 = w.tiles16;
  it.units = (p.tiles_y + EU5_UNIT_ROWS - 1) / EU5_UNIT_ROWS;
  it.start(t0, K);
  if constexpr (PAIRS) {
    int *const queue = p.wl + EU4_WL_DYN(xcd);
    const int nbatch = (w.l2_off[xcd + 1] - w.l2_off[xcd]) * w.l2_half;
    const eu5_cint rows2 = (eu5_cint)w.l2_rows + w.l2_off[xcd];
    auto take = [&]() -> int {
      int v = 0;
      if (lane0 == 0) v = atomicAdd(queue, 1);
      return v;
    };
    auto decode = [&](int j, int &ty, int &tcol) -> bool {
      if (j >= nbatch) return false;
      const int r = (int)(((unsigned long long)(unsigned)j * w.l2_magic) >> 40);
      ty = rows2[r]; tcol = 2 * (j - r * w.l2_half);
      return true;
    };
    int ty_a = 0, col_a = 0, ty_n = 0, col_n = 0;
    bool have = decode(__builtin_amdgcn_readfirstlane(take()), ty_a, col_a);
    eu5_tab8 Ta, Tb;
    if (have) eu5_load8<FAST>(p, ty_a, col_a * EU4_TW, lane0, Ta);
#pragma unroll 1
    while (have) {
      const int jn_lane = take();
      const bool second = col_a + 1 < w.tiles16;
      {
        int lane = lane0;
        asm volatile("" : "+v"(lane));
        eu5_tile<NCH, DEG, PRJ, false, FAST, true>(p, w, atab, tile, nullptr, ty_a, col_a * EU4_TW, lane, &Ta, second, ty_a,
                                                   (col_a + 1) * EU4_TW, &Tb);
      }
      const bool have_n = decode(__builtin_amdgcn_readfirstlane(jn_lane), ty_n, col_n);
      if (second) {
        int lane = lane0;
        asm volatile("" : "+v"(lane));
        eu5_tile<NCH, DEG, PRJ, false, FAST, true>(p, w, atab, tile, nullptr, ty_a, (col_a + 1) * EU4_TW, lane, &Tb, have_n, ty_n,
                                                   col_n * EU4_TW, &Ta);
      } else if (have_n) eu5_load8<FAST>(p, ty_n, col_n * EU4_TW, lane0, Ta);
      ty_a = ty_n; col_a = col_n; have = have_n;
    }
  } else {
    int plan_n = (it.done() || it.row() >= p.tiles_y) ? -2 : (PRJ == EU_SPHERICAL ? ((eu5_cint)w.tileplan)[it.row()] : -1);
#pragma unroll 1
    while (!it.done()) {
      const int tile_y = it.row(), tcol = it.col(), plan = plan_n;
      it.step();
      plan_n = (it.done() || it.row() >= p.tiles_y) ? -2 : (PRJ == EU_SPHERICAL ? ((eu5_cint)w.tileplan)[it.row()] : -1);
      if (plan == -2) continue;
      int lane = lane0;
      asm volatile("" : "+v"(lane));
      if (plan >= 0)
        eu5_tile<NCH, DEG, PRJ, PRJ == EU_SPHERICAL, FAST>(p, w, atab, tile, w.coltab + (size_t)plan * p.width * EU4_COL_FLOATS,
                                                            tile_y, tcol * EU4_TW, lane);
      else
        eu5_tile<NCH, DEG, PRJ, false, FAST>(p, w, atab, tile, nullptr, tile_y, tcol * EU4_TW, lane);
    }
  }
#ifdef EU5_STAMPS
  if (lane0 == 0 && w.stamps) {
    unsigned long long *o = w.stamps + (size_t)w.tiles16 * p.tiles_y * 8 + ((size_t)blockIdx.x * EU5_WAVES + wave) * 4;
    o[0] = ws0; o[1] = ws1; o[2] = __builtin_amdgcn_s_memtime(); o[3] = 1;
  }
#endif
}
```

### include/eu_hip.h

```cpp
#ifndef EU_HIP_H
#define EU_HIP_H

#include <stddef.h>
#include <stdint.h>

#ifdef __cplusplus
extern "C" {
#endif

typedef enum {
  EU_SPHERICAL = 0, EU_CYLINDRICAL, EU_RECTILINEAR, EU_STEREOGRAPHIC,
  EU_FISHEYE, EU_CUBEMAP, EU_BIATAN6, EU_PRJ_NONE
} eu_projection;

typedef enum {
  EU_BC_MIRROR = 0, EU_BC_PERIODIC, EU_BC_REFLECT, EU_BC_NATURAL,
  EU_BC_CONSTANT, EU_BC_ZEROPAD, EU_BC_GUESS
} eu_bc;

typedef enum {
  EU_OK = 0,
  EU_ERR_NO_DEVICE = -1,
  EU_ERR_ARGUMENT = -2,
  EU_ERR_UNSUPPORTED = -3,
  EU_ERR_MEMORY = -4,
  EU_ERR_HANDLE = -5
} eu_status;

#define EU_MAX_DEGREE 9
#define EU_MAX_TAPS 1024
#define EU_MAX_FACETS 64

typedef struct eu_facet {
  int32_t projection;
  int32_t nchannels;
  double  hfov;
  int32_t width, height;
  int32_t window_width, window_height, window_x_offset, window_y_offset;
  double  yaw, pitch, roll;
  double  brighten;
  double  step;
  int32_t has_lcp;
  double  a, b, c, h, v, s, shear_g, shear_t;
  double  tr_x, tr_y, tr_z, tp_y, tp_p, tp_r;
  int32_t mask_paint;
} eu_facet;

typedef struct eu_source eu_source;

typedef struct eu_container {
  int64_t shape[2];
  int64_t left[2], right[2];
  int64_t core[2];
} eu_container;

typedef struct eu_target {
  int32_t projection;
  int32_t width, height;
  double  x0, x1, y0, y1;
  double  yaw, pitch, roll;
  int32_t nchannels;
  int32_t ntaps;
  const float *taps;
  int32_t row_begin, row_end;
  int32_t stage;
  int32_t crop_x0, crop_y0, crop_w, crop_h;
  int32_t out_format;
  int32_t band_rows, band_count, band_index;
  int32_t synopsis;
  const eu_facet *single;
} eu_target;

int  eu_hip_layout_segments(const eu_target *trg, eu_source *const *srcs, int nsrc,
                            unsigned char *flags, int max_flags, int *seg_rows);

unsigned long long eu_hip_launch_count(void);

int  eu_hip_band_rows(int height, int band_rows, int band_count, int band_index);

enum { EU_OUT_FLOAT = 0, EU_OUT_SRGBA8 = 1 };
enum { EU_SYN_PANORAMA = 0, EU_SYN_HDR_MERGE = 1 };

int  eu_hip_device_count(void);
int  eu_hip_init(int device);
const char *eu_hip_last_error(void);

#define EU_MAX_SLOTS 16
int  eu_hip_init_devices(const int *devices, int ndevices);
int  eu_hip_device_slots(void);
int  eu_hip_render_devices(const eu_target *trg, eu_source *const *srcs, int nsrc, float *out,
                           size_t out_row_stride_bytes, int out_on_device);
int  eu_hip_device_strips(const eu_target *trg, eu_source *const *srcs, int nsrc, int *begin, int *end);

int  eu_hip_get_extent(int projection, int width, int height, double hfov,
                       double *x0x1y0y1);
double eu_hip_get_step(int projection, int width, int height, double hfov);
int  eu_hip_make_spread(int w, int h, float d, float sigma, float threshold,
                        float *taps, int max_taps);
typedef struct eu_mask_polygon { int n; const float *x; const float *y; } eu_mask_polygon;
int  eu_hip_facet_alpha(float *pixels, int width, int height, int nchannels,
                        const eu_mask_polygon *polygons, int npolygons, int crop_kind,
                        int crop_x0, int crop_x1, int crop_y0, int crop_y1, float *alpha_out);
int  eu_hip_facet_alpha_rows(int width, int height, const eu_mask_polygon *polygons, int npolygons,
                             int crop_kind, int crop_x0, int crop_x1, int crop_y0, int crop_y1,
                             int32_t *keep, int32_t *row_start, int32_t *spans, int max_spans);
typedef struct eu_facet_edit {
  const eu_mask_polygon *polygons; int32_t npolygons;
  int32_t crop_kind, crop_x0, crop_x1, crop_y0, crop_y1;
  int32_t pixel_channels;
  int32_t pixels_on_device;
} eu_facet_edit;
int  eu_hip_facet_alpha_dev(void *pixels_dev, int width, int height, int nchannels,
                            const eu_facet_edit *edit, float *alpha_out_dev, void *stream);
int  eu_hip_cubemap_metrics(int face_px, double face_fov, int support_min,
                            int tile_px, int64_t *section_px,
                            int64_t *left_frame_px, double *refc_md,
                            double *model_to_px);
int  eu_hip_container_geometry(int degree, int bc0, int bc1, int64_t w,
                               int64_t h, eu_container *out);

int  eu_hip_source_load(const eu_facet *fct, const float *pixels,
                        int spline_degree, int prefilter_degree,
                        int support_min, int tile_size, eu_source **out);
int  eu_hip_source_load_edited(const eu_facet *fct, const void *pixels, const eu_facet_edit *edit,
                               int spline_degree, int prefilter_degree, int support_min,
                               int tile_size, eu_source **out);
int  eu_hip_source_adopt(const eu_facet *fct, const float *container,
                         int spline_degree, int bc0, int bc1,
                         int support_min, int tile_size, eu_source **out);
int  eu_hip_source_alloc(const eu_facet *fct, int spline_degree,
                         int support_min, int tile_size, eu_source **out);
int  eu_hip_source_update_facet(eu_source *src, const eu_facet *fct);
int  eu_hip_source_device_ptr(const eu_source *src, void **dev_ptr,
                              size_t *nfloats);
int  eu_hip_source_download(const eu_source *src, float *container,
                            size_t nfloats);
int  eu_hip_source_info(const eu_source *src, eu_container *geom, int *nch);
int  eu_hip_source_release(eu_source *src);

int  eu_hip_render(const eu_target *trg, eu_source *const *srcs, int nsrc,
                   float *out, size_t out_row_stride_bytes, int out_on_device,
                   void *stream);
int  eu_hip_sync(void);

int  eu_hip_render_timed(const eu_target *trg, eu_source *const *srcs, int nsrc,
                         float *out_dev, size_t out_row_stride_bytes,
                         int iters, float *mean_ms);

int  eu_hip_malloc(void **p, size_t bytes);
int  eu_hip_free(void *p);
int  eu_hip_memcpy_d2h(void *dst, const void *src, size_t bytes);
int  eu_hip_memcpy_h2d(void *dst, const void *src, size_t bytes);

#ifdef __cplusplus
}
#endif
#endif
```

Measured before the change: 97810.

## Share latitude and gather work across symmetric cubemap faces and mirrored columns

Adds a host-side planner that groups tile rows whose vertical ray components and column tables match, across cubemap faces and mirrored column halves. The render5 kernel then evaluates one group per work item, computing the atan2 latitude and vertical weights once and reusing them for every member face or mirror tile. A per-tile x-extent table lets the bounding box be read precomputed instead of reduced from the columns. This aims to cut redundant transcendental and index work on symmetric cubemap layouts, at the cost of a device-to-host copy of the column tables during planning and more complex kernel control flow.

```diff
diff --git a/envutil_amd/csrc/eu_render4.hip b/envutil_amd/csrc/eu_render4.hip
--- a/envutil_amd/csrc/eu_render4.hip
+++ b/envutil_amd/csrc/eu_render4.hip
@@ -68,9 +68,11 @@
   int l2_off[9];
   int l2_half;
   unsigned long long l2_magic;
-  const int *l1_rows;
+  const int *l1_ent;
   int l1_off[9];
+  int l1_ecols;
   unsigned long long l1_magic;
+  const int *xtab;
 #ifdef EU5_STAMPS
   unsigned long long *stamps;
 #endif
@@ -78,8 +80,10 @@
 
 #ifdef EU5_STAMPS
 #define EU5_STAMP(k) do { asm volatile("" ::: "memory"); st_[k] = __builtin_amdgcn_s_memtime(); asm volatile("" ::: "memory"); } while (0)
+#define EU5_STAMP32(k) do { asm volatile("" ::: "memory"); st_[k] = (unsigned)__builtin_amdgcn_s_memtime(); asm volatile("" ::: "memory"); } while (0)
 #else
 #define EU5_STAMP(k) do { } while (0)
+#define EU5_STAMP32(k) do { } while (0)
 #endif
 
 template <int NCH, int DEG, int PRJ>
@@ -282,6 +286,7 @@
   if (vb) eu_put<NCH>(orow, xb, pxb);
 }
 
+#include "eu_share_groups.h"
 #include "eu_render5.h"
 
 template <int DEG>
@@ -364,6 +369,9 @@
   }
 }
 
+static long long eu4_followers_plan = 0, eu4_followers_last = 0;
+extern "C" unsigned long long eu_hip_share_follower_tiles(void) { return (unsigned long long)eu4_followers_last; }
+
 #ifndef EU4_DIRECT_WGS
 #define EU4_DIRECT_WGS 2048
 #endif
@@ -392,6 +400,7 @@
     }
     const int wgs = (cus / 8) * 8 * per_cu;
     if (wgs <= 0) return -1;
+    if (fast) eu4_followers_last = eu4_followers_plan;
     if (fast) hipLaunchKernelGGL((eu_render5_kernel<NCH, DEG, PRJ, true>), dim3((unsigned)wgs), dim3(64 * EU5_WAVES), 0, st, p, w);
     else hipLaunchKernelGGL((eu_render5_kernel<NCH, DEG, PRJ, false>), dim3((unsigned)wgs), dim3(64 * EU5_WAVES), 0, st, p, w);
   } else {
@@ -446,8 +455,11 @@
   int planned_rows = 0;
   int *l2_rows = nullptr; size_t l2_cap = 0;
   int l2_off[9] = {};
-  int *l1_rows = nullptr; size_t l1_cap = 0;
+  int *l1_ent = nullptr; size_t l1_cap = 0;
   int l1_off[9] = {};
+  int l1_ecols = 1;
+  int *xtab = nullptr; size_t xtab_cap = 0;
+  long long follower_tiles = 0;
   hipStream_t last_stream = nullptr;
 } g4s[EU_MAX_SLOTS];
 #define g4 (g4s[eu_current_slot()])
@@ -473,6 +485,7 @@
                                  unsigned long long plan_gen, int only_if_worth, void *stream)
 {
   eu_render_params p = *pp;
+  eu4_followers_last = 0;
   if (p.twine || p.stage != 0 || p.form >= EU_FORM_FISH || p.src.has_lcp || p.nch_out != p.nch) return 1;
   if (p.norm_mode != EU_NORM_NONE && p.norm_mode != EU_NORM_DIV) return 1;
   if (p.src.prj != EU_SPHERICAL && p.src.prj != EU_CUBEMAP && p.src.prj != EU_BIATAN6) return 1;
@@ -489,13 +502,19 @@
   if (!ensure_atab()) return -1;
   w.atab_g = g4.atab;
 
-  std::vector<unsigned char> key(sizeof(unsigned long long) + sizeof(eu_src_dev) + 8 * sizeof(int));
+  int share_mode = EU_SHARE_FACES | EU_SHARE_MIRRORS;
+  if (const char *e = getenv("EU_HIP_SHARE")) {
+    if (e[0] == '0') share_mode = 0;
+    else if (e[0] == 'm') share_mode = EU_SHARE_MIRRORS;
+    else if (e[0] == 'f') share_mode = EU_SHARE_FACES;
+  }
+  std::vector<unsigned char> key(sizeof(unsigned long long) + sizeof(eu_src_dev) + 9 * sizeof(int));
   {
     unsigned char *q = key.data();
     memcpy(q, &plan_gen, sizeof plan_gen); q += sizeof plan_gen;
     eu_src_dev sd = p.src; sd.base = nullptr;
     memcpy(q, &sd, sizeof sd); q += sizeof sd;
-    const int v[8] = { p.width, p.row_begin, p.row_end, p.band_shift, p.band_count, p.band_index, p.form, p.norm_mode };
+    const int v[9] = { p.width, p.row_begin, p.row_end, p.band_shift, p.band_count, p.band_index, p.form, p.norm_mode, share_mode };
     memcpy(q, v, sizeof v);
   }
   if (p.src.prj == EU_SPHERICAL && key != g4.key) {
@@ -561,22 +580,6 @@
         g4.l2_cap = all.size() + 1;
       }
       if (!all.empty() && hipMemcpy(g4.l2_rows, all.data(), all.size() * sizeof(int), hipMemcpyHostToDevice) != hipSuccess) return -1;
-      std::vector<int> prs[8];
-      for (int m = 0; 2 * m + 1 < p.tiles_y; m++)
-        if (tp[(size_t)2 * m] >= 0 && tp[(size_t)2 * m] == tp[(size_t)2 * m + 1]) {
-          auto &v = prs[(m / (EU5_UNIT_ROWS / 2)) & 7];
-          v.push_back(m); v.push_back(tp[(size_t)2 * m]);
-        }
-      std::vector<int> all1;
-      for (int x = 0; x < 8; x++) { g4.l1_off[x] = (int)all1.size() / 2; all1.insert(all1.end(), prs[x].begin(), prs[x].end()); }
-      g4.l1_off[8] = (int)all1.size() / 2;
-      if (g4.l1_cap < all1.size() + 2) {
-        if (g4.l1_rows) (void)hipFree(g4.l1_rows);
-        g4.l1_rows = nullptr; g4.l1_cap = 0;
-        if (hipMalloc((void **)&g4.l1_rows, (all1.size() + 2) * sizeof(int)) != hipSuccess) return -1;
-        g4.l1_cap = all1.size() + 2;
-      }
-      if (!all1.empty() && hipMemcpy(g4.l1_rows, all1.data(), all1.size() * sizeof(int), hipMemcpyHostToDevice) != hipSuccess) return -1;
     }
     for (size_t j = 0; j < plans.size() / 4; j++) {
       float *ct = g4.coltab + j * (size_t)p.width * EU4_COL_FLOATS;
@@ -587,6 +590,43 @@
       }
       if (hipGetLastError() != hipSuccess) return -1;
     }
+    {
+      const int nplans = (int)(plans.size() / 4);
+      std::vector<float> h_ct((size_t)nplans * p.width * EU4_COL_FLOATS);
+      if (nplans) {
+        if (hipStreamSynchronize(st) != hipSuccess) return -1;
+        if (hipMemcpy(h_ct.data(), g4.coltab, h_ct.size() * sizeof(float), hipMemcpyDeviceToHost) != hipSuccess) return -1;
+      }
+      std::vector<int> cm, cp;
+      for (int m = 0; 2 * m + 1 < p.tiles_y; m++)
+        if (tp[(size_t)2 * m] >= 0 && tp[(size_t)2 * m] == tp[(size_t)2 * m + 1]) { cm.push_back(m); cp.push_back(tp[(size_t)2 * m]); }
+      eu_share_input in;
+      in.width = p.width; in.tiles16 = w.tiles16; in.row_begin = p.row_begin; in.row_end = p.row_end;
+      in.band_mode = p.band_count > 1;
+      in.ncand = (int)cm.size(); in.cand_m = cm.data(); in.cand_plan = cp.data();
+      in.h_row = h_row; in.h_row_floats = h_row_floats; in.row_floats = EU_ROW_FLOATS;
+      in.coltab = nplans ? h_ct.data() : nullptr; in.col_floats = EU4_COL_FLOATS; in.nplans = nplans;
+      in.mode = share_mode; in.unit_drows = EU5_UNIT_ROWS / 2;
+      eu_share_result gr;
+      eu_share_build(in, gr);
+      if (g4.l1_cap < gr.entries.size() + 2) {
+        if (g4.l1_ent) (void)hipFree(g4.l1_ent);
+        g4.l1_ent = nullptr; g4.l1_cap = 0;
+        if (hipMalloc((void **)&g4.l1_ent, (gr.entries.size() + 2) * sizeof(int)) != hipSuccess) return -1;
+        g4.l1_cap = gr.entries.size() + 2;
+      }
+      if (!gr.entries.empty() && hipMemcpy(g4.l1_ent, gr.entries.data(), gr.entries.size() * sizeof(int), hipMemcpyHostToDevice) != hipSuccess) return -1;
+      if (g4.xtab_cap < gr.xtab.size()) {
+        if (g4.xtab) (void)hipFree(g4.xtab);
+        g4.xtab = nullptr; g4.xtab_cap = 0;
+        if (hipMalloc((void **)&g4.xtab, gr.xtab.size() * sizeof(int)) != hipSuccess) return -1;
+        g4.xtab_cap = gr.xtab.size();
+      }
+      if (hipMemcpy(g4.xtab, gr.xtab.data(), gr.xtab.size() * sizeof(int), hipMemcpyHostToDevice) != hipSuccess) return -1;
+      for (int x = 0; x < 9; x++) g4.l1_off[x] = gr.off[x];
+      g4.l1_ecols = gr.ecols;
+      g4.follower_tiles = gr.follower_tiles;
+    }
     g4.key.swap(key);
   }
   if (only_if_worth && p.src.prj == EU_SPHERICAL) {
@@ -598,9 +638,12 @@
   for (int x = 0; x < 9; x++) w.l2_off[x] = g4.l2_off[x];
   w.l2_half = (w.tiles16 + 1) / 2;
   w.l2_magic = (1ull << 40) / (unsigned long long)w.l2_half + 1;
-  w.l1_rows = g4.l1_rows;
+  w.l1_ent = g4.l1_ent;
   for (int x = 0; x < 9; x++) w.l1_off[x] = g4.l1_off[x];
-  w.l1_magic = (1ull << 40) / (unsigned long long)w.tiles16 + 1;
+  w.l1_ecols = g4.l1_ecols;
+  w.l1_magic = (1ull << 40) / (unsigned long long)w.l1_ecols + 1;
+  w.xtab = g4.xtab;
+  eu4_followers_plan = g4.follower_tiles;
   g4.last_stream = st;
 #ifdef EU5_STAMPS
   static unsigned long long *d_st = nullptr; static size_t st_cap = 0; static int dumps = 0;
diff --git a/envutil_amd/csrc/eu_render5.h b/envutil_amd/csrc/eu_render5.h
--- a/envutil_amd/csrc/eu_render5.h
+++ b/envutil_amd/csrc/eu_render5.h
@@ -483,124 +483,188 @@
   T.c0 = (eu_f2){ p.col[xac], p.col[xbc] };
 }
 
+typedef const __attribute__((address_space(4))) int *eu5_cint;
+
+__device__ __forceinline__ void eu5_load_cols(const float *ct, int xa, int xb, eu5_tab16 &T)
+{
+  const eu4_f4 *ea = (const eu4_f4 *)(ct + (size_t)xa * EU4_COL_FLOATS);
+  const eu4_f4 *eb = (const eu4_f4 *)(ct + (size_t)xb * EU4_COL_FLOATS);
+  T.a0 = ea[0]; T.a1 = ea[1]; T.b0 = eb[0]; T.b1 = eb[1];
+}
+
+__device__ __forceinline__ void eu5_y_reduce(int &mn, int &mx)
+{
+#define EU5_RED2(ctrl)                                       \
+  "v_min_i32_dpp %0, %0, %0 " ctrl "\n\t"                    \
+  "v_max_i32_dpp %1, %1, %1 " ctrl "\n\t"                    \
+  "s_nop 1\n\t"
+  asm("s_nop 1\n\t"
+      EU5_RED2("row_shr:1 row_mask:0xf bank_mask:0xf")
+      EU5_RED2("row_shr:2 row_mask:0xf bank_mask:0xf")
+      EU5_RED2("row_shr:4 row_mask:0xf bank_mask:0xf")
+      EU5_RED2("row_shr:8 row_mask:0xf bank_mask:0xf")
+      EU5_RED2("row_bcast:15 row_mask:0xa bank_mask:0xf")
+      EU5_RED2("row_bcast:31 row_mask:0xc bank_mask:0xf")
+      : "+v"(mn), "+v"(mx));
+#undef EU5_RED2
+  mn = __builtin_amdgcn_readlane(mn, 63); mx = __builtin_amdgcn_readlane(mx, 63);
+}
+
 template <int NCH, int DEG>
-__device__ __forceinline__ bool eu5_tile16h(const eu_render_params &p, const eu4_plan &w, const float *atab,
-                                            float *wtile, const eu5_tab16 &T, int tile_y, int x0, int lane,
-                                            bool have_n, const float *ct_n, int ty_n, int x0_n, eu5_tab16 &Tn)
+__device__ __forceinline__ void eu5_group16(const eu_render_params &p, const eu4_plan &w, const float *atab, float *wtile,
+                                            eu5_tab16 &T, eu5_cint ent, int n, int m0, int plan0, int tcol, int lane0,
+                                            bool have_n, int m_n, int plan_n, int tcol_n)
 {
   constexpr int order = DEG + 1;
   const eu_src_dev &s = p.src;
 #ifdef EU5_STAMPS
-  unsigned long long st_[8] = { 0, 0, 0, 0, 0, 0, 0, 0 };
-#endif
-  EU5_STAMP(0);
-  const int pr = lane & 3, rw = (lane >> 2) & 7, hf = lane >> 5;
-  const int yA = p.row_begin + tile_y * EU4_TH + rw, yB = yA + EU4_TH;
-  const bool yinA = yA < p.row_end, yinB = yB < p.row_end;
-  const int ycA = yinA ? yA : p.row_end - 1, ycB = yinB ? yB : p.row_end - 1;
-  const int xa = x0 + 8 * hf + 2 * pr, xb = xa + 1;
-  const bool vxa = xa < p.width, vxb = xb < p.width;
-  const eu4_f4 a0 = T.a0, a1 = T.a1, b0 = T.b0, b1 = T.b1;
-  const eu_f2 c0 = T.c0;
-  const eu_f2 ryA = T.B1A * c0 + T.A1A, ryB = T.B1B * c0 + T.A1B;
-  const int ixa = __float_as_int(a0.x), ixb = __float_as_int(b0.x);
-  eu_f2 wx[order];
-  const eu_f2 tx = { a0.y, b0.y };
-  if constexpr (DEG >= 2) {
-    wx[0] = (eu_f2){ a0.z, b0.z }; wx[1] = (eu_f2){ a0.w, b0.w }; wx[2] = (eu_f2){ a1.x, b1.x };
-    if constexpr (DEG == 3) wx[3] = (eu_f2){ a1.y, b1.y };
-  }
-  const eu_f2 qs = { a1.z, b1.z };
-  eu_i2 bigA = { 0, 0 }, bigB = { 0, 0 };
-  int bad = ((ixa != INT_MIN && ixb != INT_MIN) ? 0 : -1) |
-            eu5_out_of_range3(ryA.x, qs.x, ryB.x) | eu5_out_of_range3(ryA.y, qs.y, ryB.y);
-  const eu_f2 latA = eu_atan2f_2_lean(ryA, qs, atab, 1, bigA);
-  const eu_f2 latB = eu_atan2f_2_lean(ryB, qs, atab, 1, bigB);
-  bad |= bigA.x | bigA.y | bigB.x | bigB.y;
-  const float rr = s.cdiv_ok ? 0.0f : eu_rcp_refined(s.ext_h);
-  eu_f2 iA = { (float)((double)latA.x - s.tex_y0), (float)((double)latA.y - s.tex_y0) };
-  eu_f2 iB = { (float)((double)latB.x - s.tex_y0), (float)((double)latB.y - s.tex_y0) };
-  if (s.cdiv_ok) { iA = eu_div2_const(iA, s.ext_h, s.rcp_ext_h); iB = eu_div2_const(iB, s.ext_h, s.rcp_ext_h); }
-  else { iA = eu_div2_rr(iA, s.ext_h, rr); iB = eu_div2_rr(iB, s.ext_h, rr); }
-  iA = iA * s.total_h; iA = iA - .5f; iB = iB * s.total_h; iB = iB - .5f;
-  const eu_f2 gyA = eu5_gate2(iA - s.win_y_off, s.gate1, s.lower1, s.upper1);
-  const eu_f2 gyB = eu5_gate2(iB - s.win_y_off, s.gate1, s.lower1, s.upper1);
-  eu_f2 fyA, fyB;
-  if constexpr (DEG & 1) { fyA = (eu_f2){ floorf(gyA.x), floorf(gyA.y) }; fyB = (eu_f2){ floorf(gyB.x), floorf(gyB.y) }; }
-  else { fyA = (eu_f2){ roundf(gyA.x), roundf(gyA.y) }; fyB = (eu_f2){ roundf(gyB.x), roundf(gyB.y) }; }
-  const eu_f2 tyA = gyA - fyA, tyB = gyB - fyB;
-  const int iyAa = (int)fyA.x, iyAb = (int)fyA.y, iyBa = (int)fyB.x, iyBb = (int)fyB.y;
-  const bool hAa = yinA && vxa, hAb = yinA && vxb, hBa = yinB && vxa, hBb = yinB && vxb;
-
-#ifdef EU5_STAMPS
-  asm volatile("" : : "v"(iyAa), "v"(iyAb), "v"(iyBa), "v"(iyBb));
-#endif
-  EU5_STAMP(2);
-  int q0 = INT_MAX, q1 = INT_MAX, q2 = INT_MIN, q3 = INT_MIN, h0, h1, h2, h3;
-  if (hAa) { q0 = ixa; q2 = ixa; q1 = iyAa; q3 = iyAa; }
-  if (hAb) { q0 = min(q0, ixb); q2 = max(q2, ixb); q1 = min(q1, iyAb); q3 = max(q3, iyAb); }
-  if (hBa) { q0 = min(q0, ixa); q2 = max(q2, ixa); q1 = min(q1, iyBa); q3 = max(q3, iyBa); }
-  if (hBb) { q0 = min(q0, ixb); q2 = max(q2, ixb); q1 = min(q1, iyBb); q3 = max(q3, iyBb); }
-  eu5_box_reduce(q0, q1, q2, q3, h0, h1, h2, h3);
-  eu5_box bx = eu5_box_join(eu5_box_at(h0, h1, h2, h3, 31), eu5_box_at(h0, h1, h2, h3, 63));
-  bool fast = __ballot(bad != 0 && (hAa || hAb || hBa || hBb)) == 0ull;
-  if (bx.mnx != INT_MAX) {
-    const int cw = (int)(s.upper0 + 0.5f), ch = (int)(s.upper1 + 0.5f);
-    if (s.gate0 == 2 && bx.mnx < 0) fast = false;
-    if (s.gate0 != 0 && bx.mxx >= cw - 1) fast = false;
-    if (s.gate1 == 2 && bx.mny < 0) fast = false;
-    if (s.gate1 != 0 && bx.mxy >= ch - 1) fast = false;
-    if (eu5_box_fits<order>(bx) != 1) fast = false;
-  }
-  if (bx.mnx == INT_MAX || !fast) {
-    if (have_n) eu5_load16(p, ct_n, ty_n, x0_n, lane, Tn);
-    return bx.mnx == INT_MAX;
-  }
-  bx.mnx = __builtin_amdgcn_readfirstlane(bx.mnx); bx.mny = __builtin_amdgcn_readfirstlane(bx.mny);
-  bx.mxx = __builtin_amdgcn_readfirstlane(bx.mxx); bx.mxy = __builtin_amdgcn_readfirstlane(bx.mxy);
-  const unsigned lds_tile = (unsigned)(unsigned long long)(eu4_lds_void)wtile;
-  EU5_STAMP(3);
-  eu5_stage<NCH, DEG>(s, bx, lds_tile, lane);
-  eu_f2 wyA[order], wyB[order];
-  if constexpr (DEG >= 2) { eu_weights2<DEG>(s.wm, tyA, wyA); eu_weights2<DEG>(s.wm, tyB, wyB); }
-  const int ibw = bx.mxx - bx.mnx + order;
-  const int oAa = hAa ? ((iyAa - bx.mny) * ibw + (ixa - bx.mnx)) * 4 : 0, oAb = hAb ? ((iyAb - bx.mny) * ibw + (ixb - bx.mnx)) * 4 : 0;
-  const int oBa = hBa ? ((iyBa - bx.mny) * ibw + (ixa - bx.mnx)) * 4 : 0, oBb = hBb ? ((iyBb - bx.mny) * ibw + (ixb - bx.mnx)) * 4 : 0;
-  EU5_STAMP(4);
-  asm volatile("s_waitcnt vmcnt(0)" ::: "memory");
-  EU5_STAMP(5);
-  __builtin_amdgcn_sched_barrier(0);
-  eu_f2 rga, bxa, rgb, bxb;
-  eu5_taps<NCH, DEG>((eu_lptr)wtile, oAa, oAb, ibw * 4, wx, wyA, tx, tyA, rga, bxa, rgb, bxb);
-  asm volatile("" : "+v"(rga), "+v"(bxa), "+v"(rgb), "+v"(bxb));
+  unsigned st_[8] = { 0, 0, 0, 0, 0, 0, 0, 0 };
+#endif
+  EU5_STAMP32(0);
+  const eu5_cint xt = (eu5_cint)w.xtab;
+  int xmn = xt[2 * (plan0 * w.tiles16 + tcol)], xmx = xt[2 * (plan0 * w.tiles16 + tcol) + 1];
+  int iyAa, iyAb, iyBa, iyBb, bad, mny = INT_MAX, mxy = INT_MIN;
+  eu_f2 tyA, tyB;
+  bool off;
   {
-    float qa[4] = { rga.x, rga.y, bxa.x, bxa.y }, qb[4] = { rgb.x, rgb.y, bxb.x, bxb.y };
-    float *const orow = p.out + (long long)(ycA - p.row_begin) * p.out_stride;
-    if (hAa) eu_put<NCH>(orow, xa, qa);
-    if (hAb) eu_put<NCH>(orow, xb, qb);
-  }
-  EU5_STAMP(6);
-  __builtin_amdgcn_sched_barrier(0);
-  eu5_taps<NCH, DEG>((eu_lptr)wtile, oBa, oBb, ibw * 4, wx, wyB, tx, tyB, rga, bxa, rgb, bxb);
-  asm volatile("" : "+v"(rga), "+v"(bxa), "+v"(rgb), "+v"(bxb));
-  if (have_n) eu5_load16(p, ct_n, ty_n, x0_n, lane, Tn);
-  __builtin_amdgcn_sched_barrier(0);
-  {
-    float qa[4] = { rga.x, rga.y, bxa.x, bxa.y }, qb[4] = { rgb.x, rgb.y, bxb.x, bxb.y };
-    float *const orow = p.out + (long long)(ycB - p.row_begin) * p.out_stride;
-    if (hBa) eu_put<NCH>(orow, xa, qa);
-    if (hBb) eu_put<NCH>(orow, xb, qb);
-  }
-  EU5_STAMP(7);
-#ifdef EU5_STAMPS
-  if (lane == 0 && w.stamps) {
-    unsigned long long *o = w.stamps + ((size_t)tile_y * w.tiles16 + x0 / EU4_TW) * 8;
-    st_[1] = 6ull | 16ull;
+    int lane = lane0;
+    asm volatile("" : "+v"(lane));
+    const int pr = lane & 3, rw = (lane >> 2) & 7, hf = lane >> 5;
+    const int yA = p.row_begin + 2 * m0 * EU4_TH + rw, yB = yA + EU4_TH;
+    const bool yinA = yA < p.row_end, yinB = yB < p.row_end;
+    const int xa = tcol * EU4_TW + 8 * hf + 2 * pr, xb = xa + 1;
+    const bool vxa = xa < p.width, vxb = xb < p.width;
+    const eu_f2 c0 = T.c0;
+    const eu_f2 ryA = T.B1A * c0 + T.A1A, ryB = T.B1B * c0 + T.A1B;
+    const eu_f2 qs = { T.a1.z, T.b1.z };
+    eu_i2 bigA = { 0, 0 }, bigB = { 0, 0 };
+    bad = eu5_out_of_range3(ryA.x, qs.x, ryB.x) | eu5_out_of_range3(ryA.y, qs.y, ryB.y);
+    const eu_f2 latA = eu_atan2f_2_lean(ryA, qs, atab, 1, bigA);
+    const eu_f2 latB = eu_atan2f_2_lean(ryB, qs, atab, 1, bigB);
+    bad |= bigA.x | bigA.y | bigB.x | bigB.y;
+    const float rr = s.cdiv_ok ? 0.0f : __int_as_float(__builtin_amdgcn_readfirstlane(__float_as_int(eu_rcp_refined(s.ext_h))));
+    eu_f2 iA = { (float)((double)latA.x - s.tex_y0), (float)((double)latA.y - s.tex_y0) };
+    eu_f2 iB = { (float)((double)latB.x - s.tex_y0), (float)((double)latB.y - s.tex_y0) };
+    if (s.cdiv_ok) { iA = eu_div2_const(iA, s.ext_h, s.rcp_ext_h); iB = eu_div2_const(iB, s.ext_h, s.rcp_ext_h); }
+    else { iA = eu_div2_rr(iA, s.ext_h, rr); iB = eu_div2_rr(iB, s.ext_h, rr); }
+    iA = iA * s.total_h; iA = iA - .5f; iB = iB * s.total_h; iB = iB - .5f;
+    const eu_f2 gyA = eu5_gate2(iA - s.win_y_off, s.gate1, s.lower1, s.upper1);
+    const eu_f2 gyB = eu5_gate2(iB - s.win_y_off, s.gate1, s.lower1, s.upper1);
+    eu_f2 fyA, fyB;
+    if constexpr (DEG & 1) { fyA = (eu_f2){ floorf(gyA.x), floorf(gyA.y) }; fyB = (eu_f2){ floorf(gyB.x), floorf(gyB.y) }; }
+    else { fyA = (eu_f2){ roundf(gyA.x), roundf(gyA.y) }; fyB = (eu_f2){ roundf(gyB.x), roundf(gyB.y) }; }
+    tyA = gyA - fyA; tyB = gyB - fyB;
+    iyAa = (int)fyA.x; iyAb = (int)fyA.y; iyBa = (int)fyB.x; iyBb = (int)fyB.y;
+#ifdef EU5_STAMPS
+    asm volatile("" : : "v"(iyAa), "v"(iyAb), "v"(iyBa), "v"(iyBb));
+#endif
+    EU5_STAMP32(2);
+    const bool hAa = yinA && vxa, hAb = yinA && vxb, hBa = yinB && vxa, hBb = yinB && vxb;
+    int q1 = INT_MAX, q3 = INT_MIN;
+    if (hAa) { q1 = iyAa; q3 = iyAa; }
+    if (hAb) { q1 = min(q1, iyAb); q3 = max(q3, iyAb); }
+    if (hBa) { q1 = min(q1, iyBa); q3 = max(q3, iyBa); }
+    if (hBb) { q1 = min(q1, iyBb); q3 = max(q3, iyBb); }
+    eu5_y_reduce(q1, q3);
+    mny = q1; mxy = q3;
+    off = __ballot(bad != 0 && (hAa || hAb || hBa || hBb)) != 0ull;
+  }
+  EU5_STAMP32(3);
+  int mk = m0, pk = plan0;
+#pragma unroll 1
+  for (int k = 0; k < n; k++) {
+    int lane = lane0;
+    asm volatile("" : "+v"(lane));
+    const int pr = lane & 3, rw = (lane >> 2) & 7, hf = lane >> 5;
+    const bool mir = (pk & EU_SHARE_MIRROR) != 0;
+    const int tc = mir ? w.tiles16 - 1 - tcol : tcol;
+    int mk_n = 0, pk_n = 0;
+    if (k + 1 < n) { mk_n = ent[2 * k + 4]; pk_n = ent[2 * k + 5]; }
+#ifdef EU5_STAMPS
+    if (k > 0) { EU5_STAMP32(0); st_[2] = st_[0]; st_[3] = st_[0]; }
+#endif
+    eu5_box bx = { xmn, mny, xmx, mxy };
+    bool fast = !off && xmn != INT_MAX && mny != INT_MAX;
+    if (fast) {
+      const int cw = __builtin_amdgcn_readfirstlane((int)(s.upper0 + 0.5f)), ch = __builtin_amdgcn_readfirstlane((int)(s.upper1 + 0.5f));
+      if (s.gate0 == 2 && bx.mnx < 0) fast = false;
+      if (s.gate0 != 0 && bx.mxx >= cw - 1) fast = false;
+      if (s.gate1 == 2 && bx.mny < 0) fast = false;
+      if (s.gate1 != 0 && bx.mxy >= ch - 1) fast = false;
+      if (eu5_box_fits<order>(bx) != 1) fast = false;
+    }
+    const int xl = 8 * hf + 2 * pr;
+    const int xa = mir ? p.width - 1 - (tcol * EU4_TW + xl) : tc * EU4_TW + xl, xb = mir ? xa - 1 : xa + 1;
+    const int yA = p.row_begin + 2 * mk * EU4_TH + rw, yB = yA + EU4_TH;
+    const bool yinA = yA < p.row_end, yinB = yB < p.row_end;
+    const int ycA = yinA ? yA : p.row_end - 1, ycB = yinB ? yB : p.row_end - 1;
+    const bool vxa = xa < p.width, vxb = xb < p.width;
+    const bool hAa = yinA && vxa, hAb = yinA && vxb, hBa = yinB && vxa, hBb = yinB && vxb;
+    eu_f2 rga = { 0.0f, 0.0f }, bxa = { 0.0f, 0.0f }, rgb = { 0.0f, 0.0f }, bxb = { 0.0f, 0.0f };
+    if (fast) eu5_stage<NCH, DEG>(s, bx, (unsigned)(unsigned long long)(eu4_lds_void)wtile, lane);
+    const bool mir_n = (pk_n & EU_SHARE_MIRROR) != 0;
+    const int plan_k = pk_n & (EU_SHARE_MIRROR - 1);
+    const int tc_k = mir_n ? w.tiles16 - 1 - tcol : tcol;
+    int xmn_n = INT_MAX, xmx_n = INT_MIN;
+    if (k + 1 < n) { xmn_n = xt[2 * (plan_k * w.tiles16 + tc_k)]; xmx_n = xt[2 * (plan_k * w.tiles16 + tc_k) + 1]; }
+    if (fast) {
+      eu_f2 wx[order], wyA[order], wyB[order];
+      const int ixa = __float_as_int(T.a0.x), ixb = __float_as_int(T.b0.x);
+      const eu_f2 tx = { T.a0.y, T.b0.y };
+      if constexpr (DEG >= 2) {
+        wx[0] = (eu_f2){ T.a0.z, T.b0.z }; wx[1] = (eu_f2){ T.a0.w, T.b0.w }; wx[2] = (eu_f2){ T.a1.x, T.b1.x };
+        if constexpr (DEG == 3) wx[3] = (eu_f2){ T.a1.y, T.b1.y };
+        eu_weights2<DEG>(s.wm, tyA, wyA); eu_weights2<DEG>(s.wm, tyB, wyB);
+      }
+      const int ibw = bx.mxx - bx.mnx + order;
+      const int oAa = hAa ? ((iyAa - bx.mny) * ibw + (ixa - bx.mnx)) * 4 : 0, oAb = hAb ? ((iyAb - bx.mny) * ibw + (ixb - bx.mnx)) * 4 : 0;
+      const int oBa = hBa ? ((iyBa - bx.mny) * ibw + (ixa - bx.mnx)) * 4 : 0, oBb = hBb ? ((iyBb - bx.mny) * ibw + (ixb - bx.mnx)) * 4 : 0;
+      asm volatile("s_waitcnt vmcnt(0)" ::: "memory");
+      __builtin_amdgcn_sched_barrier(0);
+      eu5_taps<NCH, DEG>((eu_lptr)wtile, oAa, oAb, ibw * 4, wx, wyA, tx, tyA, rga, bxa, rgb, bxb);
+      asm volatile("" : "+v"(rga), "+v"(bxa), "+v"(rgb), "+v"(bxb));
+      {
+        float qa[4] = { rga.x, rga.y, bxa.x, bxa.y }, qb[4] = { rgb.x, rgb.y, bxb.x, bxb.y };
+        float *const orow = p.out + (long long)(ycA - p.row_begin) * p.out_stride;
+        if (hAa) eu_put<NCH>(orow, xa, qa);
+        if (hAb) eu_put<NCH>(orow, xb, qb);
+      }
+      __builtin_amdgcn_sched_barrier(0);
+      eu5_taps<NCH, DEG>((eu_lptr)wtile, oBa, oBb, ibw * 4, wx, wyB, tx, tyB, rga, bxa, rgb, bxb);
+      asm volatile("" : "+v"(rga), "+v"(bxa), "+v"(rgb), "+v"(bxb));
+    } else if (mny != INT_MAX) {
+      if (lane < 2) {
+        const int id = (2 * mk + lane) * w.tiles16 + tc;
+        const int sh = eu4_shard_of(id);
+        const int slot = atomicAdd(p.wl + EU4_WL_SHARD(sh), 1);
+        p.wl[EU4_WL_ENTRIES + (size_t)slot * EU4_SHARDS + sh] = id;
+      }
+    }
+    if (k + 1 < n) {
+      const int xa_n = mir_n ? p.width - 1 - (tcol * EU4_TW + xl) : tcol * EU4_TW + xl, xb_n = mir_n ? xa_n - 1 : xa_n + 1;
+      const int xac = xa_n < p.width ? xa_n : p.width - 1, xbc = xb_n < p.width ? xb_n : p.width - 1;
+      eu5_load_cols(w.coltab + (size_t)plan_k * p.width * EU4_COL_FLOATS, xac, xbc, T);
+    } else if (have_n) {
+      eu5_load16(p, w.coltab + (size_t)plan_n * p.width * EU4_COL_FLOATS, 2 * m_n, tcol_n * EU4_TW, lane, T);
+    }
+    __builtin_amdgcn_sched_barrier(0);
+    if (fast) {
+      float qa[4] = { rga.x, rga.y, bxa.x, bxa.y }, qb[4] = { rgb.x, rgb.y, bxb.x, bxb.y };
+      float *const orow = p.out + (long long)(ycB - p.row_begin) * p.out_stride;
+      if (hBa) eu_put<NCH>(orow, xa, qa);
+      if (hBb) eu_put<NCH>(orow, xb, qb);
+    }
+    EU5_STAMP32(7);
+#ifdef EU5_STAMPS
+    if (fast && lane == 0 && w.stamps) {
+      unsigned long long *o = w.stamps + ((size_t)(2 * mk) * w.tiles16 + tc) * 8;
+      st_[1] = (k == 0 ? 6ull : 7ull) | 16ull;
 #pragma unroll
-    for (int k = 0; k < 8; k++) o[k] = st_[k];
-  }
-#endif
-  return true;
+      for (int q = 0; q < 8; q++) o[q] = q == 1 ? st_[1] : (q == 4 || q == 5) ? 0ull : (unsigned long long)st_[q == 6 ? 7 : q] | (1ull << 32);
+    }
+#endif
+    mk = mk_n; pk = pk_n; xmn = xmn_n; xmx = xmx_n;
+  }
 }
 
 template <int UNIT>
@@ -633,7 +697,6 @@
   }
 };
 
-typedef const __attribute__((address_space(4))) int *eu5_cint;
 __device__ __forceinline__ int eu5_pair_plan(const int *tileplan, int tiles_y, int m)
 {
   if (2 * m + 1 >= tiles_y) return -1;
@@ -667,51 +730,31 @@
   const int t0 = (int)(blockIdx.x >> 3) * EU5_WAVES + wave;
   constexpr bool PAIRS = FAST && PRJ == EU_SPHERICAL;
   if constexpr (PAIRS) {
-    const int n1 = (w.l1_off[xcd + 1] - w.l1_off[xcd]) * w.tiles16;
-    const eu5_cint rows1 = (eu5_cint)w.l1_rows + 2 * w.l1_off[xcd];
+    const int n1 = (w.l1_off[xcd + 1] - w.l1_off[xcd]) * w.l1_ecols;
+    const eu5_cint ents = (eu5_cint)w.l1_ent + EU_SHARE_ENTRY_INTS * w.l1_off[xcd];
     int pos1 = t0;
-    auto seek = [&](int &m, int &tcol, int &plan) -> bool {
+    auto seek = [&](eu5_cint &e, int &n, int &m, int &plan, int &tcol) -> bool {
       if (pos1 >= n1) return false;
       const int r = (int)(((unsigned long long)(unsigned)pos1 * w.l1_magic) >> 40);
-      m = rows1[2 * r]; plan = rows1[2 * r + 1];
+      e = ents + EU_SHARE_ENTRY_INTS * r;
+      n = e[0]; m = e[2]; plan = e[3];
       const unsigned h = ((unsigned)m * 0x9E3779B1u) >> 16;
-      int c = pos1 - r * w.tiles16 + (int)((h * (unsigned)w.tiles16) >> 16);
-      if (c >= w.tiles16) c -= w.tiles16;
-      tcol = c;
+      int c = pos1 - r * w.l1_ecols + (int)((h * (unsigned)w.l1_ecols) >> 16);
+      if (c >= w.l1_ecols) c -= w.l1_ecols;
+      tcol = e[1] + c;
       pos1 += K;
       return true;
     };
-    int m_a = 0, col_a = 0, plan_a = -1, m_b = 0, col_b = 0, plan_b = -1;
-    bool have_a = seek(m_a, col_a, plan_a), have_b = false;
-    eu5_tab16 Ta, Tb;
-    if (have_a) eu5_load16(p, w.coltab + (size_t)plan_a * p.width * EU4_COL_FLOATS, 2 * m_a, col_a * EU4_TW, lane0, Ta);
-    auto fallback = [&](int m, int tcol, int lane) {
-      if (lane < 2) {
-        const int id = (2 * m + lane) * w.tiles16 + tcol;
-        const int sh = eu4_shard_of(id);
-        const int slot = atomicAdd(p.wl + EU4_WL_SHARD(sh), 1);
-        p.wl[EU4_WL_ENTRIES + (size_t)slot * EU4_SHARDS + sh] = id;
-      }
-    };
+    eu5_cint e_a = ents, e_n = ents;
+    int n_a = 0, m_a = 0, col_a = 0, plan_a = 0, n_n = 0, m_n = 0, col_n = 0, plan_n = 0;
+    bool have_a = seek(e_a, n_a, m_a, plan_a, col_a);
+    eu5_tab16 T;
+    if (have_a) eu5_load16(p, w.coltab + (size_t)plan_a * p.width * EU4_COL_FLOATS, 2 * m_a, col_a * EU4_TW, lane0, T);
 #pragma unroll 1
     while (have_a) {
-      {
-        have_b = seek(m_b, col_b, plan_b);
-        int lane = lane0;
-        asm volatile("" : "+v"(lane));
-        const float *ct_n = w.coltab + (size_t)(have_b ? plan_b : 0) * p.width * EU4_COL_FLOATS;
-        if (!eu5_tile16h<NCH, DEG>(p, w, atab, tile, Ta, 2 * m_a, col_a * EU4_TW, lane, have_b, ct_n, 2 * m_b, col_b * EU4_TW, Tb))
-          fallback(m_a, col_a, lane);
-      }
-      if (!have_b) break;
-      {
-        have_a = seek(m_a, col_a, plan_a);
-        int lane = lane0;
-        asm volatile("" : "+v"(lane));
-        const float *ct_n = w.coltab + (size_t)(have_a ? plan_a : 0) * p.width * EU4_COL_FLOATS;
-        if (!eu5_tile16h<NCH, DEG>(p, w, atab, tile, Tb, 2 * m_b, col_b * EU4_TW, lane, have_a, ct_n, 2 * m_a, col_a * EU4_TW, Ta))
-          fallback(m_b, col_b, lane);
-      }
+      const bool have_n = seek(e_n, n_n, m_n, plan_n, col_n);
+      eu5_group16<NCH, DEG>(p, w, atab, tile, T, e_a, n_a, m_a, plan_a, col_a, lane0, have_n, m_n, have_n ? plan_n : 0, col_n);
+      e_a = e_n; n_a = n_n; m_a = m_n; plan_a = plan_n; col_a = col_n; have_a = have_n;
     }
   }
 #ifdef EU5_STAMPS
diff --git a/envutil_amd/csrc/eu_share_groups.h b/envutil_amd/csrc/eu_share_groups.h
--- /dev/null
+++ b/envutil_amd/csrc/eu_share_groups.h
@@ -0,0 +1,140 @@
+#ifndef EU_SHARE_GROUPS_H
+#define EU_SHARE_GROUPS_H
+#include <climits>
+#include <cstddef>
+#include <cstring>
+#include <vector>
+
+#define EU_SHARE_MAX_MEMBERS 8
+#define EU_SHARE_ENTRY_INTS (2 + 2 * EU_SHARE_MAX_MEMBERS)
+#define EU_SHARE_MIRROR (1 << 30)
+#define EU_SHARE_FACES 1
+#define EU_SHARE_MIRRORS 2
+
+struct eu_share_input {
+  int width, tiles16;
+  int row_begin, row_end;
+  int band_mode;
+  int ncand;
+  const int *cand_m, *cand_plan;
+  const float *h_row;
+  size_t h_row_floats;
+  int row_floats;
+  const float *coltab;
+  int col_floats, nplans;
+  int mode;
+  int unit_drows;
+};
+
+struct eu_share_result {
+  std::vector<int> entries;
+  int off[9];
+  int ecols;
+  long long follower_tiles;
+  std::vector<int> xtab;
+};
+
+namespace eu_share_detail {
+inline bool is_zero_bits(float v) { unsigned u; memcpy(&u, &v, 4); return (u & 0x7fffffffu) == 0; }
+inline int ix_of(const eu_share_input &in, int plan, int x)
+{
+  int v; memcpy(&v, in.coltab + ((size_t)plan * in.width + x) * in.col_floats, 4); return v;
+}
+inline unsigned qs_of(const eu_share_input &in, int plan, int x)
+{
+  unsigned v; memcpy(&v, in.coltab + ((size_t)plan * in.width + x) * in.col_floats + 6, 4); return v;
+}
+}
+
+inline void eu_share_build(const eu_share_input &in, eu_share_result &out)
+{
+  using namespace eu_share_detail;
+  const int W = in.width, T = in.tiles16, np = in.nplans;
+  out.xtab.assign((size_t)(np > 0 ? np : 1) * T * 2, 0);
+  std::vector<char> plan_clean((size_t)(np > 0 ? np : 1), 1);
+  for (int pl = 0; pl < np; pl++)
+    for (int t = 0; t < T; t++) {
+      int mn = INT_MAX, mx = INT_MIN;
+      bool okc = true;
+      for (int x = 16 * t; x < 16 * t + 16 && x < W; x++) {
+        const int ix = ix_of(in, pl, x);
+        if (ix == INT_MIN) okc = false;
+        mn = ix < mn ? ix : mn; mx = ix > mx ? ix : mx;
+      }
+      if (!okc) { mn = INT_MAX; mx = INT_MIN; plan_clean[(size_t)pl] = 0; }
+      out.xtab[((size_t)pl * T + t) * 2] = mn; out.xtab[((size_t)pl * T + t) * 2 + 1] = mx;
+    }
+  const bool share_ok = in.mode != 0 && !in.band_mode && in.h_row && in.coltab;
+  const bool half = share_ok && (in.mode & EU_SHARE_MIRRORS) && W % 16 == 0 && T % 2 == 0;
+  out.ecols = half ? T / 2 : T;
+  out.follower_tiles = 0;
+  const int n = in.ncand;
+  std::vector<char> can((size_t)n, 0), done((size_t)n, 0);
+  std::vector<float> a1((size_t)n * 16, 0.0f);
+  for (int i = 0; share_ok && i < n; i++) {
+    const int y0 = in.row_begin + 16 * in.cand_m[i];
+    const int pl = in.cand_plan[i];
+    if (y0 + 16 > in.row_end || pl < 0 || pl >= np || !plan_clean[(size_t)pl]) continue;
+    bool ok = true;
+    for (int r = 0; r < 16 && ok; r++) {
+      const size_t fr = (size_t)(y0 + r) * in.row_floats;
+      if (fr + 6 > in.h_row_floats) { ok = false; break; }
+      const float A1 = in.h_row[fr + 1], B1 = in.h_row[fr + 4];
+      ok = is_zero_bits(B1) && !is_zero_bits(A1);
+      a1[(size_t)i * 16 + r] = A1;
+    }
+    can[(size_t)i] = ok;
+  }
+  std::vector<char> memo((size_t)(np > 0 ? np : 1) * (np > 0 ? np : 1) * 2, 0);
+  auto qs_eq = [&](int pa, int pb, int mirror) -> bool {
+    char &m = memo[((size_t)pa * np + pb) * 2 + mirror];
+    if (!m) {
+      m = 1;
+      for (int x = 0; x < W; x++)
+        if (qs_of(in, pa, x) != qs_of(in, pb, mirror ? W - 1 - x : x)) { m = 2; break; }
+    }
+    return m == 1;
+  };
+  std::vector<int> lists[8];
+  auto emit = [&](int xcd, int colbase, const std::vector<int> &mem) {
+    std::vector<int> &l = lists[xcd];
+    const size_t at = l.size();
+    l.resize(at + EU_SHARE_ENTRY_INTS, 0);
+    l[at] = (int)mem.size() / 2; l[at + 1] = colbase;
+    for (size_t k = 0; k < mem.size(); k++) l[at + 2 + k] = mem[k];
+    out.follower_tiles += (long long)(mem.size() / 2 - 1) * out.ecols;
+  };
+  for (int i = 0; i < n; i++) {
+    if (done[(size_t)i]) continue;
+    done[(size_t)i] = 1;
+    const int pi = in.cand_plan[i];
+    const bool mirrored = half && can[(size_t)i] && qs_eq(pi, pi, 1);
+    std::vector<int> faces(1, i);
+    const int max_faces = mirrored ? EU_SHARE_MAX_MEMBERS / 2 : EU_SHARE_MAX_MEMBERS;
+    if (can[(size_t)i] && (in.mode & EU_SHARE_FACES))
+      for (int j = i + 1; j < n && (int)faces.size() < max_faces; j++) {
+        if (done[(size_t)j] || !can[(size_t)j]) continue;
+        if (memcmp(&a1[(size_t)i * 16], &a1[(size_t)j * 16], 16 * sizeof(float)) != 0) continue;
+        const int pj = in.cand_plan[j];
+        if (!qs_eq(pi, pj, 0)) continue;
+        if (mirrored && !qs_eq(pi, pj, 1)) continue;
+        done[(size_t)j] = 1;
+        faces.push_back(j);
+      }
+    std::vector<int> mem;
+    for (int f : faces) {
+      mem.push_back(in.cand_m[f]); mem.push_back(in.cand_plan[f]);
+      if (mirrored) { mem.push_back(in.cand_m[f]); mem.push_back(in.cand_plan[f] | EU_SHARE_MIRROR); }
+    }
+    const int xcd = (in.cand_m[i] / (in.unit_drows > 0 ? in.unit_drows : 1)) & 7;
+    emit(xcd, 0, mem);
+    if (half && !mirrored) emit(xcd, T / 2, mem);
+  }
+  out.entries.clear();
+  for (int x = 0; x < 8; x++) {
+    out.off[x] = (int)(out.entries.size() / EU_SHARE_ENTRY_INTS);
+    out.entries.insert(out.entries.end(), lists[x].begin(), lists[x].end());
+  }
+  out.off[8] = (int)(out.entries.size() / EU_SHARE_ENTRY_INTS);
+}
+#endif
diff --git a/include/eu_hip.h b/include/eu_hip.h
--- a/include/eu_hip.h
+++ b/include/eu_hip.h
@@ -75,6 +75,8 @@
                             unsigned char *flags, int max_flags, int *seg_rows);
 
 unsigned long long eu_hip_launch_count(void);
+
+unsigned long long eu_hip_share_follower_tiles(void);
 
 int  eu_hip_band_rows(int height, int band_rows, int band_count, int band_index);
 
```

After: 105,900, median of 6. +8.3%, better.
